# qq456cvb/CanonicalVoting

Hardware: AMD Instinct MI355X
Metric: scenes/sec (80k-pt synthetic scans) (higher is better)
Workload: dtype f32

## Files before the change

canonicalvoting_amd/_lib.py:

```python
import ctypes
import os
import threading

_HERE = os.path.dirname(os.path.abspath(__file__))
LIB_PATH = os.path.join(_HERE, "_C", "libcvhip.so")

c_float_p = ctypes.POINTER(ctypes.c_float)
c_int_p = ctypes.POINTER(ctypes.c_int)
c_i32_p = ctypes.POINTER(ctypes.c_int32)
c_i64_p = ctypes.POINTER(ctypes.c_int64)
vp = ctypes.c_void_p
ABI_VERSION = 6


class CvError(RuntimeError):
    pass


class DecodeParams(ctypes.Structure):
    _fields_ = [("thresh_high", ctypes.c_float), ("thresh_low", ctypes.c_float),
                ("valid_ratio", ctypes.c_float), ("elimination", ctypes.c_int),
                ("prob_thresh", ctypes.c_float), ("elim_hi_plus1", ctypes.c_int),
                ("max_iters", ctypes.c_int), ("err_thresh", ctypes.c_double)]


class ConvDesc(ctypes.Structure):
    _fields_ = [("in_", vp), ("n_in", ctypes.c_longlong), ("in_ld", ctypes.c_int), ("cin", ctypes.c_int),
                ("weight", vp), ("K", ctypes.c_int), ("cout", ctypes.c_int), ("nbr", vp),
                ("n_out", ctypes.c_longlong), ("scale", vp), ("shift", vp), ("residual", vp),
                ("res_ld", ctypes.c_int), ("relu", ctypes.c_int), ("out", vp), ("out_ld", ctypes.c_int),
                ("flavour", ctypes.c_int), ("ws", vp), ("ws_bytes", ctypes.c_size_t), ("row_perm", vp),
                ("j_begin", ctypes.c_int), ("j_end", ctypes.c_int), ("acc_in", vp), ("acc_ld", ctypes.c_int),
                ("perm_groups", ctypes.c_int), ("plan_ent", vp), ("plan_cnt", vp),
                ("weight_packed", vp), ("weight_x6", vp), ("in2", vp), ("in2_ld", ctypes.c_int), ("cin2", ctypes.c_int),
                ("weight2_x6", vp), ("perm_has_map", ctypes.c_int), ("weight_pieces", ctypes.c_int),
                ("acc_scale", ctypes.c_float), ("range_flag", vp), ("in_hl", ctypes.c_int), ("out_hl", ctypes.c_int),
                ("res_hl", ctypes.c_int), ("split_tickets", vp), ("acc_scale_dev", vp), ("valid_words", vp)]


class SceneMaps(ctypes.Structure):
    _fields_ = [("stem", ctypes.c_longlong), ("out", ctypes.c_longlong), ("down", ctypes.c_longlong * 4),
                ("k3", ctypes.c_longlong * 5), ("up", ctypes.c_longlong * 4), ("mask_perm", ctypes.c_longlong * 5),
                ("up_perm", ctypes.c_longlong * 4), ("scratch", ctypes.c_longlong), ("bitmap", ctypes.c_longlong)]


class ScenePlanLayout(ctypes.Structure):
    _fields_ = [("cap", ctypes.c_longlong), ("perm", ctypes.c_longlong), ("inv", ctypes.c_longlong),
                ("coords", ctypes.c_longlong * 5), ("vals", ctypes.c_longlong * 5), ("counts", ctypes.c_longlong),
                ("arena", ctypes.c_longlong), ("int_words", ctypes.c_longlong), ("key_words", ctypes.c_longlong),
                ("sort_ws_bytes", ctypes.c_size_t), ("levels_ws_bytes", ctypes.c_size_t)]


NET_MAP_SLOTS, NET_PERM_SLOTS = 15, 9


class NetBuf(ctypes.Structure):
    _fields_ = [("level", ctypes.c_int), ("channels", ctypes.c_int), ("rows_level", ctypes.c_int), ("hl", ctypes.c_int)]


class NetOp(ctypes.Structure):
    _fields_ = [("in_buf", ctypes.c_int), ("in_col", ctypes.c_int), ("cin", ctypes.c_int),
                ("out_buf", ctypes.c_int), ("out_col", ctypes.c_int), ("cout", ctypes.c_int),
                ("res_buf", ctypes.c_int), ("res_col", ctypes.c_int), ("map", ctypes.c_int), ("K", ctypes.c_int),
                ("perm", ctypes.c_int), ("perm_groups", ctypes.c_int), ("relu", ctypes.c_int),
                ("weight", vp), ("scale", vp), ("shift", vp), ("weight_x6", vp), ("in2_buf", ctypes.c_int),
                ("in2_col", ctypes.c_int), ("cin2", ctypes.c_int), ("weight2_x6", vp), ("weight_pieces", ctypes.c_int), ("acc_scale", ctypes.c_float)]


class NetModelParams(ctypes.Structure):
    _fields_ = [("weight_x6", vp), ("weight2_x6", vp), ("scale", vp), ("shift", vp), ("acc_scale", ctypes.c_float),
                ("reserved", ctypes.c_int * 3)]


class SceneDesc(ctypes.Structure):
    _fields_ = [("d_coords4", vp), ("n", ctypes.c_longlong), ("d_feats", vp), ("feats_ld", ctypes.c_int), ("d_points", vp),
                ("res", ctypes.c_float), ("num_rots", ctypes.c_int), ("ops", vp), ("n_ops", ctypes.c_int), ("bufs", vp),
                ("n_bufs", ctypes.c_int), ("stem_k", ctypes.c_int), ("mask_groups", ctypes.c_int),
                ("masked_min_rows", ctypes.c_longlong), ("max_channels", ctypes.c_int),
                ("use_range_flag", ctypes.c_int),
                ("d_out_feats", vp), ("out_ld", ctypes.c_int), ("out_channels", ctypes.c_int), ("nclasses", ctypes.c_int),
                ("log_scale", ctypes.c_int), ("d_xyz_in", vp), ("d_scale_in", vp), ("d_prob_in", vp), ("d_class_in", vp),
                ("vote_algo", ctypes.c_int), ("decode", DecodeParams), ("max_candidates", ctypes.c_int),
                ("nms_threshold", ctypes.c_double), ("d_ws", vp), ("ws_bytes", ctypes.c_size_t), ("d_grids", vp),
                ("grid_capacity_floats", ctypes.c_size_t), ("h_pinned", vp), ("pinned_bytes", ctypes.c_size_t),
                ("h_cand_idx", vp), ("h_verdict", vp), ("h_boxes", vp), ("h_scores", vp), ("h_classes", vp), ("h_pick", vp),
                ("adaptive_split", ctypes.c_int), ("events", vp * 5),
                ("conv_split_target", ctypes.c_int), ("vote_part_records", ctypes.c_int), ("peak_quotients", ctypes.c_int)]


MAX_CATEGORIES = 16


class SceneSeparateDesc(ctypes.Structure):
    _fields_ = [("d_coords4", vp), ("n", ctypes.c_longlong), ("d_feats", vp), ("feats_ld", ctypes.c_int), ("d_points", vp),
                ("res", ctypes.c_float), ("num_rots", ctypes.c_int), ("num_models", ctypes.c_int),
                ("ops", vp), ("n_ops", vp), ("bufs", vp), ("n_bufs", vp),
                ("stem_k", ctypes.c_int), ("mask_groups", ctypes.c_int), ("masked_min_rows", ctypes.c_longlong),
                ("max_channels", ctypes.c_int), ("use_range_flag", ctypes.c_int),
                ("d_out_feats", vp), ("out_ld", ctypes.c_int), ("out_channels", ctypes.c_int), ("log_scale", ctypes.c_int),
                ("d_xyz_in", vp), ("d_scale_in", vp), ("d_prob_in", vp), ("vote_algo", ctypes.c_int), ("decode", DecodeParams),
                ("max_candidates", ctypes.c_int), ("nms_threshold", ctypes.c_double), ("d_ws", vp), ("ws_bytes", ctypes.c_size_t),
                ("h_pinned", vp), ("pinned_bytes", ctypes.c_size_t), ("h_cand_idx", vp), ("h_verdict", vp), ("h_boxes", vp),
                ("h_scores", vp), ("h_det_cat", vp), ("h_det_box", vp), ("events", vp * 5),
                ("conv_split_target", ctypes.c_int), ("vote_part_records", ctypes.c_int),
                ("models_per_pass", ctypes.c_int), ("d_model_params", vp)]


class SceneSeparateResult(ctypes.Structure):
    _fields_ = [("n_cand", ctypes.c_int * MAX_CATEGORIES), ("n_boxes", ctypes.c_int * MAX_CATEGORIES),
                ("truncated", ctypes.c_int * MAX_CATEGORIES), ("n_det", ctypes.c_int), ("range_flag", ctypes.c_int),
                ("duplicates", ctypes.c_int), ("out_of_window", ctypes.c_int), ("dims", ctypes.c_int * 3),
                ("corner", ctypes.c_float * 3), ("level_rows", ctypes.c_longlong * 5), ("needed_ws_bytes", ctypes.c_size_t),
                ("d_grid_obj", vp), ("d_grid_rot", vp), ("d_grid_scale", vp), ("d_xyz", vp), ("d_scale", vp), ("d_prob", vp),
                ("host_us", ctypes.c_float * 4)]


class PackJob(ctypes.Structure):
    _fields_ = [("w", vp), ("wp", vp), ("K", ctypes.c_int), ("cin", ctypes.c_int), ("cout", ctypes.c_int), ("trans", ctypes.c_int),
                ("scale_log2", ctypes.c_int), ("reserved", ctypes.c_int)]


class SceneResult(ctypes.Structure):
    _fields_ = [("n_cand", ctypes.c_int), ("n_boxes", ctypes.c_int), ("n_det", ctypes.c_int), ("truncated", ctypes.c_int),
                ("range_flag", ctypes.c_int), ("duplicates", ctypes.c_int), ("out_of_window", ctypes.c_int),
                ("scenes_in_flight", ctypes.c_int), ("dims", ctypes.c_int * 3), ("corner", ctypes.c_float * 3), ("level_rows", ctypes.c_longlong * 5),
                ("needed_ws_bytes", ctypes.c_size_t), ("needed_grid_floats", ctypes.c_size_t),
                ("d_grid_obj", vp), ("d_grid_rot", vp), ("d_grid_scale", vp), ("d_xyz", vp), ("d_scale", vp),
                ("d_prob", vp), ("d_class", vp), ("host_us", ctypes.c_float * 4)]


MAX_SCENES = 16


class DecodeSceneJob(ctypes.Structure):
    _fields_ = [("d_grid_obj", vp), ("d_grid_rot", vp), ("d_grid_scale", vp), ("dims", ctypes.c_int * 3),
                ("corner", ctypes.c_float * 3), ("row0", ctypes.c_int64), ("n", ctypes.c_int64)]


class ScenesDesc(ctypes.Structure):
    _fields_ = [("scene", SceneDesc), ("num_scenes", ctypes.c_int)]


class ScenesResult(ctypes.Structure):
    _fields_ = [("n_cand", ctypes.c_int * MAX_SCENES), ("n_boxes", ctypes.c_int * MAX_SCENES), ("n_det", ctypes.c_int * MAX_SCENES),
                ("truncated", ctypes.c_int * MAX_SCENES), ("dims", ctypes.c_int * 3 * MAX_SCENES),
                ("corner", ctypes.c_float * 3 * MAX_SCENES), ("row0", ctypes.c_longlong * MAX_SCENES),
                ("rows", ctypes.c_longlong * MAX_SCENES), ("d_grid_obj", vp * MAX_SCENES), ("d_grid_rot", vp * MAX_SCENES),
                ("d_grid_scale", vp * MAX_SCENES), ("range_flag", ctypes.c_int), ("duplicates", ctypes.c_int),
                ("out_of_window", ctypes.c_int), ("scenes_in_flight", ctypes.c_int), ("level_rows", ctypes.c_longlong * 5),
                ("needed_ws_bytes", ctypes.c_size_t), ("needed_grid_floats", ctypes.c_size_t),
                ("d_xyz", vp), ("d_scale", vp), ("d_prob", vp), ("d_class", vp), ("host_us", ctypes.c_float * 4)]


GATHER_MAX_JOBS = 8


class GatherJob(ctypes.Structure):
    _fields_ = [("d_src", vp), ("src_ld", ctypes.c_longlong), ("d_dst", vp), ("dst_ld", ctypes.c_longlong),
                ("width", ctypes.c_int), ("recentre_from", ctypes.c_int)]


class ScanRowsDesc(ctypes.Structure):
    _fields_ = [("d_coords4", vp), ("d_index", vp), ("n", ctypes.c_longlong), ("m_points", ctypes.c_longlong),
                ("d_points", vp), ("points_ld", ctypes.c_longlong), ("d_rgb", vp), ("d_owner", vp),
                ("d_minv", vp), ("d_model_scale", vp), ("d_model_cls", vp), ("n_models", ctypes.c_int),
                ("d_colour", vp), ("d_jitter", vp), ("n_clouds", ctypes.c_int),
                ("use_xyz", ctypes.c_int), ("recentre", ctypes.c_int),
                ("d_feats", vp), ("feats_ld", ctypes.c_longlong), ("d_xyz", vp), ("xyz_ld", ctypes.c_longlong),
                ("d_scale", vp), ("scale_ld", ctypes.c_longlong), ("d_cls", vp), ("cls_ld", ctypes.c_longlong)]


class SymLossDesc(ctypes.Structure):
    _fields_ = [("d_out", vp), ("n_rows", ctypes.c_longlong), ("ld", ctypes.c_longlong),
                ("d_rows", vp), ("d_pseg", vp), ("n_points", ctypes.c_longlong),
                ("d_seg_ptr", vp), ("d_pose_ptr", vp), ("d_tgt_ptr", vp), ("n_segments", ctypes.c_int), ("n_jobs", ctypes.c_int),
                ("d_targets", vp), ("n_targets", ctypes.c_longlong),
                ("d_urow", vp), ("d_uptr", vp), ("d_upoint", vp), ("n_urows", ctypes.c_int),
                ("w", ctypes.c_float * 3), ("xyz_factor", ctypes.c_float),
                ("d_loss", vp), ("d_pose_loss", vp), ("d_best", vp), ("d_seg_loss", vp),
                ("d_grad_loss", vp), ("d_grad", vp), ("grad_ld", ctypes.c_longlong),
                ("d_ws", vp), ("ws_bytes", ctypes.c_size_t)]


class RowLossDesc(ctypes.Structure):
    _fields_ = [("d_out", vp), ("n_rows", ctypes.c_longlong), ("ld", ctypes.c_longlong),
                ("d_labels", vp), ("d_xyz_labels", vp), ("d_scale_labels", vp),
                ("heads", ctypes.c_int), ("n_logits", ctypes.c_int), ("xyz_col", ctypes.c_int), ("scale_col", ctypes.c_int),
                ("logit_col", ctypes.c_int), ("obj_lo", ctypes.c_longlong), ("obj_hi", ctypes.c_longlong),
                ("with_xyz", ctypes.c_int), ("log_scale", ctypes.c_int), ("gather", ctypes.c_int), ("empty", ctypes.c_int),
                ("w", ctypes.c_float * 3), ("xyz_factor", ctypes.c_float), ("scale_factor", ctypes.c_float),
# ... 315 lines not shown
```

canonicalvoting_amd/csrc/conv_hd.hip:

```cpp
#include "cv_common.h"

#include <algorithm>

#include "sparse_conv_common.h"

using namespace cvsc;

namespace {

constexpr int hd_lds_bytes(int NB, int NW, int NSTG) {
    return NSTG * (NW * 4096 + 2 * NB * 32 * 64) + NW * 32 * 4 + (WP_NPRE + 1) * NW * 32 * 4 + NW * 4 + (HL_MAX_UNITS + 4) * 2;
}
constexpr int hd_blocks(int NB, int NW, int NSTG) {
    const int b = (160 * 1024) / hd_lds_bytes(NB, NW, NSTG);
    return b * NW > 32 ? 32 / NW : (b < 1 ? 1 : b);
}
template <int NB, int NW, int NSTG, class... MA>
__global__ __launch_bounds__(NW * 64, (hd_blocks(NB, NW, NSTG) * NW + 3) / 4) void conv_hd(ConvArgs a, MA... ma) {
    const unsigned by = model_enter(a, blockIdx.y, ma...);
    static_assert(NSTG == 2 || NSTG == 3, "two or three ring stages");
    constexpr int TMv = NW * 32, THv = NW * 64;
    constexpr int A_BYTES = NW * 4096, B_BYTES = 2 * NB * 32 * 64, STAGE = A_BYTES + B_BYTES;
    constexpr int B_INSTR = B_BYTES / 1024;
    constexpr int B_PER_WAVE = (B_INSTR + NW - 1) / NW;
    constexpr int EP_BYTES = NW * 32 * EP_LD * 4;
    static_assert(EP_BYTES <= NSTG * STAGE, "the epilogue tile aliases the ring");
    constexpr int OFF_ROWS = NSTG * STAGE, OFF_NBR = OFF_ROWS + TMv * 4, OFF_MASK = OFF_NBR + (WP_NPRE + 1) * TMv * 4,
                  OFF_UNITS = OFF_MASK + NW * 4,
                  LDS_TOTAL = OFF_UNITS + (HL_MAX_UNITS + 4) * 2;
    static_assert(LDS_TOTAL == hd_lds_bytes(NB, NW, NSTG) && LDS_TOTAL <= 160 * 1024, "LDS budget");
    __shared__ __attribute__((aligned(1024))) unsigned char lds[LDS_TOTAL];
    unsigned char* const sm = lds;
    int* const rows_s = reinterpret_cast<int*>(lds + OFF_ROWS);
    int (*const nbr_all)[TMv] = reinterpret_cast<int (*)[TMv]>(lds + OFF_NBR);
    unsigned* const wave_mask = reinterpret_cast<unsigned*>(lds + OFF_MASK);
    unsigned short* const units_s = reinterpret_cast<unsigned short*>(lds + OFF_UNITS);
    const int tid = threadIdx.x, lane = tid & 63, wave = tid >> 6;
    const int n0 = by * (NB * 32);
    const long long tile_id = tile_of(a);
    const int half = lane >> 5, l31 = lane & 31;
    const int nj = a.j_end - a.j_begin;
    const int nch = a.cin / KC;
    int u_lo, u_hi;
    if (a.perm_per_split) {
        u_lo = (int)((long long)nj * blockIdx.z / a.splits) * nch;
        u_hi = (int)((long long)nj * (blockIdx.z + 1) / a.splits) * nch;
    } else {
        u_lo = (int)((long long)nj * nch * blockIdx.z / a.splits);
        u_hi = (int)((long long)nj * nch * (blockIdx.z + 1) / a.splits);
    }
    const int j_first = a.j_begin + u_lo / nch, j_last = a.j_begin + (u_hi - 1) / nch;
    const int njl = u_hi > u_lo ? j_last - j_first + 1 : 0;
    const int nch2 = a.in2 ? a.cin2 / KC : 0;

    const int* perm = a.row_perm ? a.row_perm + (a.perm_per_split ? (long long)blockIdx.z * a.n_out : 0) : nullptr;
    if (tid < TMv) {
        const long long t = tile_id * TMv + tid;
        const int row = t < a.n_out ? (perm ? perm[t] : (int)t) : -1;
        rows_s[tid] = row;
        if (a.in2) nbr_all[njl][tid] = row;
    }
    {
        unsigned m = 0u;
        const int jg0 = a.j_begin + (int)((long long)nj * blockIdx.z / a.splits);
        for (int e = tid; e < njl * TMv; e += THv) {
            const int jj = e / TMv, t = e - jj * TMv;
            const long long pos = tile_id * TMv + t;
            int v = -1;
            if (pos < a.n_out) {
                if (a.nbr_perm) {
                    v = a.nbr_perm[((long long)blockIdx.z * a.n_out + pos) * a.nbr_perm_w + (j_first + jj - jg0)];
                } else {
                    const int row = perm ? perm[pos] : (int)pos;
                    v = a.nbr ? a.nbr[(long long)row * a.K + j_first + jj] : row;
                }
            }
            nbr_all[jj][t] = v;
            if (v >= 0) m |= 1u << jj;
        }
#pragma unroll
        for (int off = 32; off > 0; off >>= 1) m |= __shfl_xor(m, off);
        if (lane == 0) wave_mask[wave] = m;
    }
    __syncthreads();
    unsigned lm = 0u;
#pragma unroll
    for (int w = 0; w < NW; ++w) lm |= wave_mask[w];
    if (wave == 0) {
        const int n_first = u_hi - u_lo, n_second = nch2 > (int)blockIdx.z ? (nch2 - (int)blockIdx.z + a.splits - 1) / a.splits : 0;
        int cnt = 0;
        for (int base = 0; base < n_first + n_second; base += 64) {
            const int e = base + lane;
            int code = -1;
            if (e < n_first) {
                const int u = u_lo + e, q = u / nch;
                const int jj = a.j_begin + q - j_first;
                if ((lm >> jj) & 1u) code = (jj << 8) | (u - q * nch);
            } else if (e < n_first + n_second) {
                code = (njl << 8) | ((int)blockIdx.z + (e - n_first) * a.splits);
            }
            const unsigned long long bal = __ballot(code >= 0);
            if (code >= 0) units_s[cnt + __popcll(bal & ((1ull << lane) - 1ull))] = (unsigned short)code;
            cnt += __popcll(bal);
        }
        if (lane == 0) units_s[HL_MAX_UNITS] = (unsigned short)cnt;
    }
    __syncthreads();
    const int n_units = __builtin_amdgcn_readfirstlane((int)units_s[HL_MAX_UNITS]);
    if (n_units == 0 && a.gvalid) return;

    f32x16 acc[NB];
#pragma unroll
    for (int nb = 0; nb < NB; ++nb)
#pragma unroll
        for (int r = 0; r < 16; ++r) acc[nb][r] = 0.f;

    int b_src[B_PER_WAVE];
#pragma unroll
    for (int i = 0; i < B_PER_WAVE; ++i) {
        const int t = wave + i * NW;
        const int f = t * 64 + lane;
        const int pl = f / (NB * 32 * 4), rem = f - pl * (NB * 32 * 4);
        const int col = rem >> 2, slot = rem & 3;
        const int gc = min(n0 + col, a.cout - 1);
        b_src[i] = (pl * a.cout + gc) * 32 + ((slot ^ ((col >> 2) & 3)) << 3);
    }
    const unsigned slab_words = 2u * (unsigned)a.cout * 32u;
    const unsigned in_row_bytes = (unsigned)a.in_ld * 4u, in2_row_bytes = (unsigned)a.in2_ld * 4u;
    const unsigned char* const in_b = reinterpret_cast<const unsigned char*>(a.in);
    const unsigned char* const in2_b = reinterpret_cast<const unsigned char*>(a.in2);
    const int a_row = lane >> 3;
    unsigned a_piece[4];
#pragma unroll
    for (int q = 0; q < 4; ++q) a_piece[q] = (unsigned)(((lane & 7) ^ (((8 * q + a_row) >> 1) & 7)) << 4);

    bool live[NSTG];
#pragma unroll
    for (int q = 0; q < NSTG; ++q) live[q] = false;

    auto issue = [&](auto S, int k) -> int {
        constexpr int st = decltype(S)::value;
        const int code = __builtin_amdgcn_readfirstlane((int)units_s[k]);
        const int jj = code >> 8, c = code & 255;
        const bool second = jj == njl;
        int n_issued = 0;
        int src[4];
        bool any = false;
#pragma unroll
        for (int q = 0; q < 4; ++q) {
            src[q] = nbr_all[jj][wave * 32 + 8 * q + a_row];
            any |= src[q] >= 0;
        }
        const bool lv = __any(any);
        live[st] = lv;
        if (lv) {
            const unsigned rb_ = second ? in2_row_bytes : in_row_bytes;
            const unsigned char* const base = (second ? in2_b : in_b) + (unsigned)(c * 128);
#pragma unroll
            for (int q = 0; q < 4; ++q) {
                const unsigned char* g = src[q] >= 0 ? base + ((unsigned)src[q] * rb_ + a_piece[q]) : g_zero_chunk + a_piece[q];
                lds_dma16(g, sm + st * STAGE + wave * 4096 + q * 1024);
            }
            n_issued += 4;
        }
        const unsigned short* slab = second ? a.wp6_2 + (size_t)c * slab_words
                                            : a.wp6 + (size_t)((j_first + jj) * nch + c) * slab_words;
#pragma unroll
        for (int i = 0; i < B_PER_WAVE; ++i) {
            const int t = wave + i * NW;
            if (t < B_INSTR) {
                lds_dma16(slab + b_src[i], sm + st * STAGE + A_BYTES + t * 1024);
                ++n_issued;
            }
        }
        return n_issued;
    };
    const unsigned lds0 = (unsigned)(size_t)(lds_ptr_t)lds;
    const int bswz = (l31 >> 2) & 3, a_g = (l31 >> 1) & 7;
    unsigned a_off[4], b_off[2];
#pragma unroll
    for (int kk = 0; kk < 4; ++kk) a_off[kk] = lds0 + (unsigned)(wave * 4096 + l31 * 128 + (((2 * kk + half) ^ a_g) << 4));
#pragma unroll
    for (int ks = 0; ks < 2; ++ks) b_off[ks] = lds0 + (unsigned)(A_BYTES + l31 * 64 + (((2 * ks + half) ^ bswz) << 4));
    auto compute = [&](auto S) {
        constexpr int st = decltype(S)::value;
#pragma unroll
        for (int ks = 0; ks < 2; ++ks) {
            const unsigned aa0 = a_off[ks] + st * STAGE, aa1 = a_off[2 + ks] + st * STAGE, ab = b_off[ks] + st * STAGE;
            u32x4v A0, A1, B0[NB], B1[NB];
            hd_read_frags<NB>(aa0, aa1, ab, A0, A1, B0, B1);
            const f16x8 a0 = __builtin_bit_cast(f16x8, A0), a1 = __builtin_bit_cast(f16x8, A1);
#pragma unroll
            for (int nb = 0; nb < NB; ++nb) {
                const f16x8 b0 = __builtin_bit_cast(f16x8, B0[nb]), b1 = __builtin_bit_cast(f16x8, B1[nb]);
                acc[nb] = __builtin_amdgcn_mfma_f32_32x32x16_f16(a0, b1, acc[nb], 0, 0, 0);
                acc[nb] = __builtin_amdgcn_mfma_f32_32x32x16_f16(a1, b0, acc[nb], 0, 0, 0);
                acc[nb] = __builtin_amdgcn_mfma_f32_32x32x16_f16(a0, b0, acc[nb], 0, 0, 0);
            }
        }
    };
    typedef std::integral_constant<int, 0> S0;
    typedef std::integral_constant<int, 1> S1;
    typedef std::integral_constant<int, 2> S2;
    if constexpr (NSTG == 3) {
        int pend1 = 0;
        if (n_units > 0) issue(S0{}, 0);
        if (n_units > 1) pend1 = issue(S1{}, 1);
        auto step = [&](auto S, auto SP, int k) {
            constexpr int st = decltype(S)::value;
            wait_vmcnt_dyn(__builtin_amdgcn_readfirstlane(k + 1 < n_units ? pend1 : 0));
            __builtin_amdgcn_s_barrier();
            if (k + 2 < n_units) pend1 = issue(SP, k + 2);
            else pend1 = 0;
            if (live[st]) compute(S);
        };
#pragma unroll 1
        for (int k = 0; k < n_units; k += 3) {
            step(S0{}, S2{}, k);
            if (k + 1 >= n_units) break;
            step(S1{}, S0{}, k + 1);
            if (k + 2 >= n_units) break;
            step(S2{}, S1{}, k + 2);
        }
    } else {
        if (n_units > 0) issue(S0{}, 0);
        auto step = [&](auto S, auto SN, int k) {
            constexpr int st = decltype(S)::value;
            wait_vmcnt_le<0>();
            __builtin_amdgcn_s_barrier();
            if (k + 1 < n_units) issue(SN, k + 1);
            if (live[st]) compute(S);
        };
#pragma unroll 1
        for (int k = 0; k < n_units; k += 2) {
            step(S0{}, S1{}, k);
            if (k + 1 >= n_units) break;
            step(S1{}, S0{}, k + 1);
        }
    }
    wait_vmcnt_le<0>();
    __syncthreads();
    model_epilogue(a, blockIdx.y, ma...);
    {
        const float sc = a.acc_scale_dev ? a.acc_scale * *a.acc_scale_dev : a.acc_scale;
#pragma unroll
        for (int nb = 0; nb < NB; ++nb)
#pragma unroll
            for (int r = 0; r < 16; ++r) acc[nb][r] *= sc;
    }
    float (*ep)[EP_LD] = reinterpret_cast<float (*)[EP_LD]>(sm + wave * 32 * EP_LD * 4);
    ConvArgs ae = a;
    ae.tickets = nullptr;
#pragma unroll
    for (int nb = 0; nb < NB; ++nb) epilogue_store_wide(ae, acc[nb], rows_s + wave * 32, n0 + nb * 32, lane, ep);
}


}

void cvsc::launch_conv_hd(const ConvArgs& a, int nb, int hd_shape, const ModelArgs* ma, dim3 grid, hipStream_t st) {
    with_nb<3>(nb, [&](auto nbc) {
        constexpr int NB = decltype(nbc)::value;
        if (hd_shape == 1) with_models(ma, [&](auto... m) { conv_hd<NB, 4, 2, decltype(m)...><<<grid, 256, 0, st>>>(a, m...); });
        else if (hd_shape == 2) with_models(ma, [&](auto... m) { conv_hd<NB, 8, 2, decltype(m)...><<<grid, 512, 0, st>>>(a, m...); });
        else with_models(ma, [&](auto... m) { conv_hd<NB, 8, 3, decltype(m)...><<<grid, 512, 0, st>>>(a, m...); });
    });
}
```

canonicalvoting_amd/csrc/conv_hl.hip:

```cpp
#include "cv_common.h"

#include <algorithm>

#include "sparse_conv_common.h"

using namespace cvsc;

namespace {

constexpr int hl_blocks(int NB) { return NB <= 3 ? 4 : 2; }
template <int NB, class... MA>
__global__ __attribute__((amdgpu_waves_per_eu(hl_blocks(NB), 8)))
__launch_bounds__(THREADS, hl_blocks(NB)) void conv_hl(ConvArgs a, MA... ma) {
    const unsigned by = model_enter(a, blockIdx.y, ma...);
    constexpr int NS = 2, NW = THREADS / 64;
    constexpr int B_BYTES = 2 * NB * 32 * 64, EP_BYTES = NW * 32 * EP_LD * 4;
    constexpr int SM_BYTES = NS * B_BYTES > EP_BYTES ? NS * B_BYTES : EP_BYTES;
    __shared__ __attribute__((aligned(16))) unsigned char sm[SM_BYTES];
    __shared__ int rows_s[TM];
    __shared__ int nbr_all[WP_NPRE + 1][TM];
    __shared__ unsigned wave_mask[NW];
    __shared__ unsigned short units_s[HL_MAX_UNITS + 4];
    const int tid = threadIdx.x, lane = tid & 63, wave = tid >> 6;
    const int n0 = by * (NB * 32);
    const long long tile_id = tile_of(a);
    const int half = lane >> 5, l31 = lane & 31;
    const int nj = a.j_end - a.j_begin;
    const int nch = a.cin / KC;
    int u_lo, u_hi;
    if (a.perm_per_split) {
        u_lo = (int)((long long)nj * blockIdx.z / a.splits) * nch;
        u_hi = (int)((long long)nj * (blockIdx.z + 1) / a.splits) * nch;
    } else {
        u_lo = (int)((long long)nj * nch * blockIdx.z / a.splits);
        u_hi = (int)((long long)nj * nch * (blockIdx.z + 1) / a.splits);
    }
    const int j_first = a.j_begin + u_lo / nch, j_last = a.j_begin + (u_hi - 1) / nch;
    const int njl = u_hi > u_lo ? j_last - j_first + 1 : 0;
    const int nch2 = a.in2 ? a.cin2 / KC : 0;

    const int* perm = a.row_perm ? a.row_perm + (a.perm_per_split ? (long long)blockIdx.z * a.n_out : 0) : nullptr;
    if (tid < TM) {
        const long long t = tile_id * TM + tid;
        const int row = t < a.n_out ? (perm ? perm[t] : (int)t) : -1;
        rows_s[tid] = row;
        if (a.in2) nbr_all[njl][tid] = row;
    }
    {
        unsigned m = 0u;
        const int jg0 = a.j_begin + (int)((long long)nj * blockIdx.z / a.splits);
        for (int e = tid; e < njl * TM; e += THREADS) {
            const int jj = e / TM, t = e - jj * TM;
            const long long pos = tile_id * TM + t;
            int v = -1;
            if (pos < a.n_out) {
                if (a.nbr_perm) {
                    v = a.nbr_perm[((long long)blockIdx.z * a.n_out + pos) * a.nbr_perm_w + (j_first + jj - jg0)];
                } else {
                    const int row = perm ? perm[pos] : (int)pos;
                    v = a.nbr ? a.nbr[(long long)row * a.K + j_first + jj] : row;
                }
            }
            nbr_all[jj][t] = v;
            if (v >= 0) m |= 1u << jj;
        }
#pragma unroll
        for (int off = 32; off > 0; off >>= 1) m |= __shfl_xor(m, off);
        if (lane == 0) wave_mask[wave] = m;
    }
    __syncthreads();
    unsigned lm = 0u;
#pragma unroll
    for (int w = 0; w < NW; ++w) lm |= wave_mask[w];
    if (wave == 0) {
        const int n_first = u_hi - u_lo, n_second = nch2 > (int)blockIdx.z ? (nch2 - (int)blockIdx.z + a.splits - 1) / a.splits : 0;
        int cnt = 0;
        for (int base = 0; base < n_first + n_second; base += 64) {
            const int e = base + lane;
            int code = -1;
            if (e < n_first) {
                const int u = u_lo + e, q = u / nch;
                const int jj = a.j_begin + q - j_first;
                if ((lm >> jj) & 1u) code = (jj << 8) | (u - q * nch);
            } else if (e < n_first + n_second) {
                code = (njl << 8) | ((int)blockIdx.z + (e - n_first) * a.splits);
            }
            const unsigned long long bal = __ballot(code >= 0);
            if (code >= 0) units_s[cnt + __popcll(bal & ((1ull << lane) - 1ull))] = (unsigned short)code;
            cnt += __popcll(bal);
        }
        if (lane == 0) units_s[HL_MAX_UNITS] = (unsigned short)cnt;
    }
    __syncthreads();
    const int n_units = __builtin_amdgcn_readfirstlane((int)units_s[HL_MAX_UNITS]);
    if (n_units == 0 && a.gvalid) return;

    f32x16 acc[NB];
#pragma unroll
    for (int nb = 0; nb < NB; ++nb)
#pragma unroll
        for (int r = 0; r < 16; ++r) acc[nb][r] = 0.f;

    constexpr int B_U4 = 2 * NB * 32 * 4;
    constexpr int B_PER = (B_U4 + THREADS - 1) / THREADS;
    int b_src[B_PER], b_dst[B_PER];
#pragma unroll
    for (int i = 0; i < B_PER; ++i) {
        const int f = tid + i * THREADS;
        const int p = f / (NB * 32 * 4), rem = f - p * (NB * 32 * 4);
        const int col = rem >> 2, ch = rem & 3;
        b_src[i] = (f < B_U4 && n0 + col < a.cout) ? (p * a.cout + n0 + col) * 32 + ch * 8 : -1;
        b_dst[i] = f < B_U4 ? (p * NB * 32 + col) * 64 + ((ch ^ ((col >> 2) & 3)) << 4) : -1;
    }
    const unsigned slab_words = 2u * (unsigned)a.cout * 32u;
    const int my_row = wave * 32 + l31;
    const unsigned in_row_bytes = (unsigned)a.in_ld * 4u, in2_row_bytes = (unsigned)a.in2_ld * 4u;
    const unsigned char* const in_b = reinterpret_cast<const unsigned char*>(a.in);
    const unsigned char* const in2_b = reinterpret_cast<const unsigned char*>(a.in2);

    uint4 ra[NS][4], rb[NS][B_PER];
    bool live[NS];
#pragma unroll
    for (int q = 0; q < NS; ++q) live[q] = false;
    auto load = [&](auto S, int k) {
        constexpr int sl = decltype(S)::value;
        const int code = __builtin_amdgcn_readfirstlane((int)units_s[k]);
        const int jj = code >> 8, c = code & 255;
        const bool second = jj == njl;
        const int src = nbr_all[jj][my_row];
        live[sl] = __any(src >= 0);
        if (src >= 0) {
            const unsigned off = (unsigned)src * (second ? in2_row_bytes : in_row_bytes) + (unsigned)(c * 128 + half * 16);
            const unsigned char* p = (second ? in2_b : in_b) + off;
            ra[sl][0] = *reinterpret_cast<const uint4*>(p);
            ra[sl][1] = *reinterpret_cast<const uint4*>(p + 32);
            ra[sl][2] = *reinterpret_cast<const uint4*>(p + 64);
            ra[sl][3] = *reinterpret_cast<const uint4*>(p + 96);
        } else {
#pragma unroll
            for (int q = 0; q < 4; ++q) ra[sl][q] = make_uint4(0u, 0u, 0u, 0u);
        }
        const unsigned short* slab = second ? a.wp6_2 + (size_t)c * slab_words
                                            : a.wp6 + (size_t)((j_first + jj) * nch + c) * slab_words;
#pragma unroll
        for (int i = 0; i < B_PER; ++i)
            rb[sl][i] = b_src[i] >= 0 ? *reinterpret_cast<const uint4*>(slab + b_src[i]) : make_uint4(0u, 0u, 0u, 0u);
    };
    auto stage_b = [&](auto S, int toff) {
        constexpr int sl = decltype(S)::value;
#pragma unroll
        for (int i = 0; i < B_PER; ++i)
            if (b_dst[i] >= 0) *reinterpret_cast<uint4*>(sm + toff + b_dst[i]) = rb[sl][i];
    };
    const int b_rd = l31 * 64;
    const int bswz = (l31 >> 2) & 3;
    auto compute = [&](auto S, int toff) {
        constexpr int sl = decltype(S)::value;
        const unsigned char* Bb = sm + toff + b_rd;
        uint4 (&fa)[4] = ra[sl];
#pragma unroll
        for (int ks = 0; ks < 2; ++ks) {
            const int piece = ((2 * ks + half) ^ bswz) << 4;
            const f16x8 a0 = __builtin_bit_cast(f16x8, fa[ks]), a1 = __builtin_bit_cast(f16x8, fa[2 + ks]);
#pragma unroll
            for (int nb = 0; nb < NB; ++nb) {
                const f16x8 b0 = *reinterpret_cast<const f16x8*>(Bb + nb * 32 * 64 + piece);
                const f16x8 b1 = *reinterpret_cast<const f16x8*>(Bb + (NB * 32 + nb * 32) * 64 + piece);
                acc[nb] = __builtin_amdgcn_mfma_f32_32x32x16_f16(a0, b1, acc[nb], 0, 0, 0);
                acc[nb] = __builtin_amdgcn_mfma_f32_32x32x16_f16(a1, b0, acc[nb], 0, 0, 0);
                acc[nb] = __builtin_amdgcn_mfma_f32_32x32x16_f16(a0, b0, acc[nb], 0, 0, 0);
                if constexpr (NB >= 3) asm volatile("" ::: "memory");
            }
        }
    };
    typedef std::integral_constant<int, 0> S0;
    typedef std::integral_constant<int, 1> S1;
    if (n_units > 0) load(S0{}, 0);
    if (n_units > 1) load(S1{}, 1);
    if (n_units > 0) stage_b(S0{}, 0);
    auto step = [&](auto S, auto SN, int k) {
        constexpr int sl = decltype(S)::value;
        __syncthreads();
        if (k + 1 < n_units) stage_b(SN, decltype(SN)::value * B_BYTES);
        if (live[sl]) compute(S, sl * B_BYTES);
        if (k + 2 < n_units) load(S, k + 2);
    };
#pragma unroll 1
    for (int k = 0; k < n_units; k += 2) {
        step(S0{}, S1{}, k);
        if (k + 1 >= n_units) break;
        step(S1{}, S0{}, k + 1);
    }
    __syncthreads();
    model_epilogue(a, blockIdx.y, ma...);
    {
        const float sc = a.acc_scale_dev ? a.acc_scale * *a.acc_scale_dev : a.acc_scale;
#pragma unroll
        for (int nb = 0; nb < NB; ++nb)
#pragma unroll
            for (int r = 0; r < 16; ++r) acc[nb][r] *= sc;
    }
    float (*ep)[EP_LD] = reinterpret_cast<float (*)[EP_LD]>(sm + wave * 32 * EP_LD * 4);
#pragma unroll
    for (int nb = 0; nb < NB; ++nb) epilogue_store_wide(a, acc[nb], rows_s + wave * 32, n0 + nb * 32, lane, ep);
    if (a.splits > 1 && a.tickets) {
        __shared__ int last_flag;
        asm volatile("s_waitcnt vmcnt(0)" ::: "memory");
        __syncthreads();
        int* ticket = a.tickets + tile_id * gridDim.y + by;
        if (tid == 0) {
            const int old = __hip_atomic_fetch_add(ticket, 1, __ATOMIC_RELAXED, __HIP_MEMORY_SCOPE_AGENT);
            last_flag = old == a.splits - 1;
            if (last_flag) __builtin_amdgcn_fence(__ATOMIC_ACQUIRE, "agent");
        }
        __syncthreads();
        if (!last_flag) return;
        if (tid == 0) *ticket = 0;
        const long long plane = a.n_out * (long long)a.cout;
#pragma unroll
        for (int nb = 0; nb < NB; ++nb) {
            const int col = n0 + nb * 32 + (lane & 7) * 4;
            if (col >= a.cout) continue;
#pragma unroll
            for (int it = 0; it < 4; ++it) {
                const int row = rows_s[wave * 32 + (lane >> 3) + 8 * it];
                if (row < 0) continue;
                const float* p = a.partial + (long long)row * a.cout + col;
                float4 sq[4];
#pragma unroll
                for (int q = 0; q < 4; ++q) sq[q] = make_float4(0.f, 0.f, 0.f, 0.f);
                for (int k0 = 0; k0 < a.splits; k0 += 4) {
#pragma unroll
                    for (int q = 0; q < 4; ++q)
                        if (k0 + q < a.splits) {
                            const float4 v = *reinterpret_cast<const float4*>(p + (long long)(k0 + q) * plane);
                            sq[q].x += v.x; sq[q].y += v.y; sq[q].z += v.z; sq[q].w += v.w;
                        }
                }
                const float4 x = make_float4(sq[0].x + sq[1].x + sq[2].x + sq[3].x, sq[0].y + sq[1].y + sq[2].y + sq[3].y,
                                             sq[0].z + sq[1].z + sq[2].z + sq[3].z, sq[0].w + sq[1].w + sq[2].w + sq[3].w);
                epilogue_apply4(a, row, col, x);
            }
        }
    }
}

}

void cvsc::launch_conv_hl(const ConvArgs& a, int nb, const ModelArgs* ma, dim3 grid, hipStream_t st) {
    with_nb<4>(nb, [&](auto nbc) {
        constexpr int NB = decltype(nbc)::value;
        with_models(ma, [&](auto... m) { conv_hl<NB, decltype(m)...><<<grid, THREADS, 0, st>>>(a, m...); });
    });
}
```

canonicalvoting_amd/csrc/conv_rows.hip:

```cpp
#include "cv_common.h"

#include <algorithm>

#include "sparse_conv_common.h"

using namespace cvsc;

namespace {

template <int NB, bool VEC>
__global__ __launch_bounds__(THREADS) void conv_rows(ConvArgs a) {
    __shared__ float A_s[KC][A_LD];
    __shared__ float B_s[KC][NB * 32];
    __shared__ int nbr_s[TM];
    __shared__ int rows_s[TM];
    __shared__ __attribute__((aligned(16))) float ep_s[4][32][EP_LD];
    const int tid = threadIdx.x, lane = tid & 63, wave = tid >> 6;
    const int n0 = blockIdx.y * (NB * 32);

    if (tid < TM) {
        const long long t = tile_of(a) * TM + tid;
        const int* perm = a.row_perm ? a.row_perm + (a.perm_per_split ? (long long)blockIdx.z * a.n_out : 0) : nullptr;
        rows_s[tid] = t < a.n_out ? (perm ? perm[t] : (int)t) : -1;
    }
    __syncthreads();

    f32x16 acc[NB];
#pragma unroll
    for (int nb = 0; nb < NB; ++nb)
#pragma unroll
        for (int r = 0; r < 16; ++r) acc[nb][r] = 0.f;

    auto compute = [&]() {
#pragma unroll
        for (int kk = 0; kk < KC; kk += 2) {
            const float av = A_s[kk + (lane >> 5)][wave * 32 + (lane & 31)];
#pragma unroll
            for (int nb = 0; nb < NB; ++nb) {
                const float bv = B_s[kk + (lane >> 5)][nb * 32 + (lane & 31)];
                acc[nb] = __builtin_amdgcn_mfma_f32_32x32x2f32(av, bv, acc[nb], 0, 0, 0);
            }
        }
    };

    const int nj = a.j_end - a.j_begin;
    if (VEC) {
        const int a_col = (tid & 7) * 4;
        const int a_row = tid >> 3;
        constexpr int B_F4 = KC * NB * 32 / 4;
        constexpr int B_PER = (B_F4 + THREADS - 1) / THREADS;
        const int nch = a.cin / KC;
        int u_lo, u_hi;
        if (a.perm_per_split) {
            u_lo = (int)((long long)nj * blockIdx.z / a.splits) * nch;
            u_hi = (int)((long long)nj * (blockIdx.z + 1) / a.splits) * nch;
        } else {
            u_lo = (int)((long long)nj * nch * blockIdx.z / a.splits);
            u_hi = (int)((long long)nj * nch * (blockIdx.z + 1) / a.splits);
        }
        const int j_first = a.j_begin + u_lo / nch, j_last = a.j_begin + (u_hi - 1) / nch;
        for (int j = j_first; j <= j_last && u_hi > u_lo; ++j) {
            const int kc_begin = (j == j_first ? u_lo % nch : 0) * KC;
            const int kc_end = (j == j_last ? (u_hi - 1) % nch + 1 : nch) * KC;
            int my = -1;
            if (tid < TM) {
                const int row = rows_s[tid];
                if (row >= 0) {
                    if (a.nbr_perm) {
                        const long long tile_id = (long long)gridDim.x - 1 - blockIdx.x;
                        my = a.nbr_perm[((long long)blockIdx.z * a.n_out + tile_id * TM + tid) * a.nbr_perm_w +
                                        (j - (a.j_begin + (int)((long long)nj * blockIdx.z / a.splits)))];
                    } else
                        my = a.nbr ? a.nbr[(long long)row * a.K + j] : row;
                }
                nbr_s[tid] = my;
            }
            if (!__syncthreads_or(my >= 0)) continue;
            const bool wave_live = __any(nbr_s[wave * 32 + (lane & 31)] >= 0);
            float4 ra[4], rb[B_PER];
            auto load = [&](int kc) {
#pragma unroll
                for (int i = 0; i < 4; ++i) {
                    const int src = nbr_s[a_row + 32 * i];
                    ra[i] = src >= 0 ? *reinterpret_cast<const float4*>(a.in + (long long)src * a.in_ld + kc + a_col)
                                     : make_float4(0.f, 0.f, 0.f, 0.f);
                }
#pragma unroll
                for (int i = 0; i < B_PER; ++i) {
                    const int f = tid + i * THREADS;
                    if (f < B_F4) {
                        const int kr = f / (NB * 8), c4 = (f % (NB * 8)) * 4;
                        const int col = n0 + c4;
                        const float* wp = a.w + ((long long)j * a.cin + kc + kr) * a.cout + col;
                        if (col + 3 < a.cout) rb[i] = *reinterpret_cast<const float4*>(wp);
                        else {
                            rb[i].x = col < a.cout ? wp[0] : 0.f;
                            rb[i].y = col + 1 < a.cout ? wp[1] : 0.f;
                            rb[i].z = col + 2 < a.cout ? wp[2] : 0.f;
                            rb[i].w = 0.f;
                        }
                    }
                }
            };
            auto stage = [&]() {
#pragma unroll
                for (int i = 0; i < 4; ++i) {
                    const int r = a_row + 32 * i;
                    A_s[a_col + 0][r] = ra[i].x; A_s[a_col + 1][r] = ra[i].y;
                    A_s[a_col + 2][r] = ra[i].z; A_s[a_col + 3][r] = ra[i].w;
                }
#pragma unroll
                for (int i = 0; i < B_PER; ++i) {
                    const int f = tid + i * THREADS;
                    if (f < B_F4) {
                        const int kr = f / (NB * 8), c4 = (f % (NB * 8)) * 4;
                        *reinterpret_cast<float4*>(&B_s[kr][c4]) = rb[i];
                    }
                }
            };
            load(kc_begin);
            for (int kc = kc_begin; kc < kc_end; kc += KC) {
                __syncthreads();
                stage();
                __syncthreads();
                if (kc + KC < kc_end) load(kc + KC);
                if (wave_live) compute();
            }
            __syncthreads();
        }
    } else {
        const int k0 = a.j_begin * a.cin, ktot = a.j_end * a.cin;
        const int nchunks = (ktot - k0 + KC - 1) / KC;
        const int c_lo = (int)((long long)nchunks * blockIdx.z / a.splits);
        const int c_hi = (int)((long long)nchunks * (blockIdx.z + 1) / a.splits);
        for (int kc = k0 + c_lo * KC; kc < k0 + c_hi * KC; kc += KC) {
            __syncthreads();
            for (int e = tid; e < KC * TM; e += THREADS) {
                const int kk = e / TM, r = e % TM;
                const int kf = kc + kk;
                float v = 0.f;
                const int row = rows_s[r];
                if (kf < ktot && row >= 0) {
                    const int j = kf / a.cin, c = kf - j * a.cin;
                    const int src = a.nbr ? a.nbr[(long long)row * a.K + j] : row;
                    if (src >= 0) v = a.in[(long long)src * a.in_ld + c];
                }
                A_s[kk][r] = v;
            }
            for (int e = tid; e < KC * NB * 32; e += THREADS) {
                const int kr = e / (NB * 32), c = e % (NB * 32);
                const int kf = kc + kr, col = n0 + c;
                B_s[kr][c] = (kf < ktot && col < a.cout) ? a.w[(long long)kf * a.cout + col] : 0.f;
            }
            __syncthreads();
            compute();
        }
    }
    if (a.wide) {
#pragma unroll
        for (int nb = 0; nb < NB; ++nb)
            epilogue_store_wide(a, acc[nb], rows_s + wave * 32, n0 + nb * 32, lane, ep_s[wave]);
    } else {
#pragma unroll
        for (int nb = 0; nb < NB; ++nb)
            epilogue_store(a, acc[nb], rows_s + wave * 32, n0 + nb * 32 + (lane & 31), lane);
    }
}

}

void cvsc::launch_conv_rows(const ConvArgs& a, int nb, bool vec, dim3 grid, hipStream_t st) {
    with_nb<4>(nb, [&](auto nbc) {
        constexpr int NB = decltype(nbc)::value;
        if (vec) conv_rows<NB, true><<<grid, THREADS, 0, st>>>(a);
        else conv_rows<NB, false><<<grid, THREADS, 0, st>>>(a);
    });
}
```

canonicalvoting_amd/csrc/conv_rows_wp.hip:

```cpp
#include "cv_common.h"

#include <algorithm>

#include "sparse_conv_common.h"

using namespace cvsc;

namespace {


template <int NB, int P, int NPRE = WP_NPRE>
__global__ __launch_bounds__(THREADS, (NB >= 3 ? 3 : NB == 2 ? 4 : 5)) void conv_rows_wp(ConvArgs a) {
    constexpr int A_BYTES = P * TM * 64, B_BYTES = P * NB * 32 * 64, EP_BYTES = 4 * 32 * EP_LD * 4;
    constexpr int SM_BYTES = A_BYTES + 2 * B_BYTES > EP_BYTES ? A_BYTES + 2 * B_BYTES : EP_BYTES;
    __shared__ __attribute__((aligned(16))) unsigned char sm[SM_BYTES];
    __shared__ int rows_s[TM];
    __shared__ int nbr_all[NPRE + 1][TM];
    __shared__ unsigned live_mask;
    unsigned char* const A_h = sm;
    unsigned char* const B_h = sm + A_BYTES;
    const int tid = threadIdx.x, lane = tid & 63, wave = tid >> 6;
    const int n0 = blockIdx.y * (NB * 32);

    const long long tile_id = tile_of(a);
// ... 43 lines not shown
                    acc[nb] = __builtin_amdgcn_mfma_f32_32x32x16_f16(a0, b1, acc[nb], 0, 0, 0);
                    acc[nb] = __builtin_amdgcn_mfma_f32_32x32x16_f16(a1, b0, acc[nb], 0, 0, 0);
                    acc[nb] = __builtin_amdgcn_mfma_f32_32x32x16_f16(a0, b0, acc[nb], 0, 0, 0);
                }
            }
        }
    };

    const int nj = a.j_end - a.j_begin;
    const int a_col = (lane & 7) * 4;
    const int a_row = wave * 32 + (lane >> 3);
    constexpr int B_U4 = P * NB * 32 * 4;
    constexpr int B_PER = (B_U4 + THREADS - 1) / THREADS;
    const int nch = a.cin / KC;
    int u_lo, u_hi;
    if (a.perm_per_split) {
        u_lo = (int)((long long)nj * blockIdx.z / a.splits) * nch;
        u_hi = (int)((long long)nj * (blockIdx.z + 1) / a.splits) * nch;
    } else {
        u_lo = (int)((long long)nj * nch * blockIdx.z / a.splits);
        u_hi = (int)((long long)nj * nch * (blockIdx.z + 1) / a.splits);
    }
    const int j_first = a.j_begin + u_lo / nch, j_last = a.j_begin + (u_hi - 1) / nch;
    const int njl = u_hi > u_lo ? j_last - j_first + 1 : 0;
    auto map_entry = [&](int t, int j) {
        const int row = rows_s[t];
        if (row < 0) return -1;
        if (a.nbr_perm) {
            return a.nbr_perm[((long long)blockIdx.z * a.n_out + tile_id * TM + t) * a.nbr_perm_w +
                              (j - (a.j_begin + (int)((long long)nj * blockIdx.z / a.splits)))];
        }
        return a.nbr ? a.nbr[(long long)row * a.K + j] : row;
    };
    {
        unsigned m = 0u;
        for (int e = tid; e < njl * TM; e += THREADS) {
            const int jj = e / TM, t = e - jj * TM;
            const int v = map_entry(t, j_first + jj);
            nbr_all[jj][t] = v;
            if (v >= 0) m |= 1u << jj;
        }
#pragma unroll
        for (int off = 32; off > 0; off >>= 1) m |= __shfl_xor(m, off);
        if (lane == 0 && m) atomicOr(&live_mask, m);
        if (a.in2 && tid < TM) nbr_all[njl][tid] = rows_s[tid];
    }
    __syncthreads();
    const unsigned lm = live_mask;

    float4 ra[4];
    uint4 rb[B_PER];
    float in_max = 0.f;
    const int c_first = u_lo - (u_lo / nch) * nch, c_last = u_hi > u_lo ? (u_hi - 1) - ((u_hi - 1) / nch) * nch + 1 : 0;
    auto skip_dead = [&](int& j, int& c) {
#pragma unroll 1
        while (j <= j_last && !((lm >> (j - j_first)) & 1u)) { ++j; c = 0; }
    };
    const int nch2 = a.in2 ? a.cin2 / KC : 0;
    const int j_second = j_last + 1, j_done = j_last + 2;
    auto advance = [&](int& j, int& c) {
        if (j <= j_last) {
            if (++c >= (j == j_last ? c_last : nch)) { ++j; c = 0; skip_dead(j, c); }
            if (j > j_last) { j = j_second; c = blockIdx.z; }
        } else {
            c += a.splits;
        }
        if (j == j_second && c >= nch2) j = j_done;
    };
    auto load = [&](int j, int c) {
        const bool second = j == j_second;
        const int kc = c * KC;
        const int* nb_j = nbr_all[j - j_first];
        const float* src_base = second ? a.in2 : a.in;
        const int src_ld = second ? a.in2_ld : a.in_ld;
#pragma unroll
        for (int i = 0; i < 4; ++i) {
            const int src = nb_j[a_row + 8 * i];
            ra[i] = src >= 0 ? *reinterpret_cast<const float4*>(src_base + (long long)src * src_ld + kc + a_col)
                             : make_float4(0.f, 0.f, 0.f, 0.f);
        }
        const unsigned short* slab = second ? a.wp6_2 + (long long)c * P * a.cout * 32
                                            : a.wp6 + (long long)(j * nch + c) * P * a.cout * 32;
#pragma unroll
        for (int i = 0; i < B_PER; ++i) {
            const int f = tid + i * THREADS;
            if (f < B_U4) {
                const int p = f / (NB * 32 * 4), rem = f - p * (NB * 32 * 4);
                const int col = rem >> 2, ch = rem & 3;
                rb[i] = (n0 + col < a.cout)
                            ? *reinterpret_cast<const uint4*>(slab + ((long long)p * a.cout + n0 + col) * 32 + ch * 8)
                            : make_uint4(0u, 0u, 0u, 0u);
            }
        }
    };
    auto stage = [&](unsigned char* Bb) {
#pragma unroll
        for (int i = 0; i < 4; ++i) {
            const int r = a_row + 8 * i;
            unsigned h0 = 0, m0 = 0, l0 = 0, h1 = 0, m1 = 0, l1 = 0;
            unsigned char* dst = A_h + r * 64 + ((((a_col >> 3) ^ ((r >> 2) & 3))) << 4) + ((a_col & 7) << 1);
            if constexpr (P == 1) {
                *reinterpret_cast<uint2*>(dst) = make_uint2(cvt_pk_bf16(ra[i].x, ra[i].y), cvt_pk_bf16(ra[i].z, ra[i].w));
            } else if constexpr (P == 3) {
                split3(ra[i].x, ra[i].y, h0, m0, l0);
                split3(ra[i].z, ra[i].w, h1, m1, l1);
                *reinterpret_cast<uint2*>(dst) = make_uint2(h0, h1);
                *reinterpret_cast<uint2*>(dst + TM * 64) = make_uint2(m0, m1);
                *reinterpret_cast<uint2*>(dst + 2 * TM * 64) = make_uint2(l0, l1);
            } else {
                in_max = fmaxf(fmaxf(in_max, fmaxf(fabsf(ra[i].x), fabsf(ra[i].y))), fmaxf(fabsf(ra[i].z), fabsf(ra[i].w)));
                split2h(ra[i].x, ra[i].y, h0, l0);
                split2h(ra[i].z, ra[i].w, h1, l1);
                *reinterpret_cast<uint2*>(dst) = make_uint2(h0, h1);
                *reinterpret_cast<uint2*>(dst + TM * 64) = make_uint2(l0, l1);
            }
        }
#pragma unroll
        for (int i = 0; i < B_PER; ++i) {
            const int f = tid + i * THREADS;
            if (f < B_U4) {
                const int p = f / (NB * 32 * 4), rem = f - p * (NB * 32 * 4);
                const int col = rem >> 2, ch = rem & 3;
                *reinterpret_cast<uint4*>(Bb + (p * NB * 32 + col) * 64 + ((ch ^ ((col >> 2) & 3)) << 4)) = rb[i];
            }
        }
    };
    int j = j_first, c = c_first, buf = 0;
    if (njl > 0) skip_dead(j, c); else j = j_last + 1;
    if (j > j_last) { j = j_second; c = blockIdx.z; if (c >= nch2) j = j_done; }
    if (j < j_done) load(j, c);
#pragma unroll 1
    while (j < j_done) {
        unsigned char* Bb = B_h + buf * B_BYTES;
        stage(Bb);
        __syncthreads();
        const bool wave_live = __any(nbr_all[j - j_first][wave * 32 + l31] >= 0);
        advance(j, c);
        if (j < j_done) load(j, c);
        if (wave_live) compute(Bb);
        buf ^= 1;
    }
    __syncthreads();
    if constexpr (P == 2) {
        if (in_max > 65000.f && a.range_flag) *a.range_flag = 1;
        const float k = a.acc_scale;
#pragma unroll
        for (int nb = 0; nb < NB; ++nb)
#pragma unroll
            for (int r = 0; r < 16; ++r) acc[nb][r] *= k;
    }
    float (*ep)[EP_LD] = reinterpret_cast<float (*)[EP_LD]>(sm + wave * 32 * EP_LD * 4);
    if (a.wide) {
#pragma unroll
        for (int nb = 0; nb < NB; ++nb) epilogue_store_wide(a, acc[nb], rows_s + wave * 32, n0 + nb * 32, lane, ep);
    } else {
#pragma unroll
        for (int nb = 0; nb < NB; ++nb)
            epilogue_store(a, acc[nb], rows_s + wave * 32, n0 + nb * 32 + (lane & 31), lane);
    }
}

}

void cvsc::launch_conv_rows_wp(const ConvArgs& a, int nb, int pieces, bool npre_big, dim3 grid, hipStream_t st) {
    with_nb<4>(nb, [&](auto nbc) {
        constexpr int NB = decltype(nbc)::value;
        if (npre_big) {
            if (pieces == 2) conv_rows_wp<NB, 2, WP_NPRE_BIG><<<grid, THREADS, 0, st>>>(a);
            else if (pieces == 1) conv_rows_wp<NB, 1, WP_NPRE_BIG><<<grid, THREADS, 0, st>>>(a);
            else conv_rows_wp<NB, 3, WP_NPRE_BIG><<<grid, THREADS, 0, st>>>(a);
        } else {
            if (pieces == 2) conv_rows_wp<NB, 2><<<grid, THREADS, 0, st>>>(a);
            else if (pieces == 1) conv_rows_wp<NB, 1><<<grid, THREADS, 0, st>>>(a);
            else conv_rows_wp<NB, 3><<<grid, THREADS, 0, st>>>(a);
        }
    });
}
```

canonicalvoting_amd/csrc/net_exec.cpp:

```cpp
#include <algorithm>
#include <mutex>
#include <unordered_map>
#include <vector>

#include "cv_common.h"

namespace {

struct Slot { char* ptr; int ld; long long rows; int ext; };

struct NetModels {
    int K;
    const void* const* const* ext_ptr;
    size_t arena_stride, ws_stride;
    const cv_net_model_params* d_params;
    int params_ld;
};

int net_run(const cv_net_op* ops, int n_ops, const cv_net_buf* bufs, int n_bufs, const long long* level_rows, int n_levels,
            void* d_arena, size_t arena_bytes, const void* const* ext_ptr, const int* ext_ld, const int32_t* const* maps,
            int n_maps, const int32_t* const* perms, int n_perms, void* d_ws, size_t ws_bytes, int32_t* range_flag,
            const NetModels* nm, bool plan_maps, void* stream);

}
// ... 288 lines not shown
    cv_net_model_params* t = static_cast<cv_net_model_params*>(h_params);
    for (int k = 0; k < n_ops; ++k)
        for (int m = 0; m < K; ++m) {
            const cv_net_op& o = ops[m][k];
            t[(size_t)k * K + m] = {o.weight_x6, o.weight2_x6, o.scale, o.shift, o.acc_scale != 0.f ? o.acc_scale : 1.f, {0, 0, 0}};
        }
    return CV_OK;
}

size_t cv_net_models_arena_bytes(const cv_net_buf* bufs, int n_bufs, const long long* level_rows, int n_levels, int K) {
    if (K < 1 || K > CV_MAX_CATEGORIES) return 0;
    return (size_t)K * cv_net_arena_bytes(bufs, n_bufs, level_rows, n_levels);
}

size_t cv_net_models_workspace_bytes(size_t one_model_bytes, int K) {
    if (K < 1 || K > CV_MAX_CATEGORIES) return 0;
    return (size_t)(K - 1) * cv_align_up(one_model_bytes, 256) + one_model_bytes;
}

int cv_net_run_models_f32(const cv_net_op* const* ops, const cv_net_buf* const* bufs, int n_ops, int n_bufs, int K,
                          const long long* level_rows, int n_levels, void* d_arena, size_t arena_bytes,
                          const void* const* const* ext_ptr, const int* ext_ld, const int32_t* const* maps, int n_maps,
                          const int32_t* const* perms, int n_perms, void* d_ws, size_t ws_bytes, int32_t* range_flag,
                          const void* d_params, int params_ld, void* stream) {
    return cv_net_run_models_ex(ops, bufs, n_ops, n_bufs, K, level_rows, n_levels, d_arena, arena_bytes, ext_ptr, ext_ld, maps, n_maps,
                                perms, n_perms, d_ws, ws_bytes, range_flag, d_params, params_ld,  false, stream);
}

}

int cv_net_run_models_ex(const cv_net_op* const* ops, const cv_net_buf* const* bufs, int n_ops, int n_bufs, int K,
                         const long long* level_rows, int n_levels, void* d_arena, size_t arena_bytes,
                         const void* const* const* ext_ptr, const int* ext_ld, const int32_t* const* maps, int n_maps,
                         const int32_t* const* perms, int n_perms, void* d_ws, size_t ws_bytes, int32_t* range_flag,
                         const void* d_params, int params_ld, bool plan_maps, void* stream) {
    CV_REQUIRE(K >= 1 && K <= CV_MAX_CATEGORIES, CV_EINVAL, "number of models out of range (%d, 1..%d)", K, CV_MAX_CATEGORIES);
    CV_REQUIRE(ops && bufs && level_rows && d_arena && ext_ptr && n_ops > 0 && n_bufs > 0 && n_levels > 0, CV_EINVAL,
               "bad network program arguments");
    CV_REQUIRE(d_params, CV_EINVAL, "null model parameter table (cv_net_models_params_fill)");
    CV_REQUIRE(params_ld >= K, CV_EINVAL, "params_ld (%d) is smaller than the number of models (%d)", params_ld, K);
    for (int m = 0; m < K; ++m)
        CV_REQUIRE(ops[m] && bufs[m] && ext_ptr[m], CV_EINVAL, "model %d: null program, buffer list or pointer table", m);
    for (int m = 1; m < K; ++m) {
        for (int i = 0; i < n_bufs; ++i) {
            const cv_net_buf &x = bufs[0][i], &y = bufs[m][i];
            CV_REQUIRE(x.level == y.level && x.channels == y.channels && x.rows_level == y.rows_level && x.hl == y.hl, CV_EINVAL,
                       "buffer %d of model %d differs from model 0's: the programs are not structurally identical", i, m);
        }
        for (int k = 0; k < n_ops; ++k) {
            const cv_net_op &x = ops[0][k], &y = ops[m][k];
            const bool same = x.in_buf == y.in_buf && x.in_col == y.in_col && x.cin == y.cin && x.out_buf == y.out_buf &&
                              x.out_col == y.out_col && x.cout == y.cout && x.res_buf == y.res_buf && x.res_col == y.res_col &&
                              x.map == y.map && x.K == y.K && x.perm == y.perm && x.perm_groups == y.perm_groups &&
                              x.relu == y.relu && x.in2_buf == y.in2_buf && x.in2_col == y.in2_col && x.cin2 == y.cin2 &&
                              x.weight_pieces == y.weight_pieces && !x.weight == !y.weight && !x.scale == !y.scale &&
                              !x.shift == !y.shift && !x.weight_x6 == !y.weight_x6 && !x.weight2_x6 == !y.weight2_x6;
            CV_REQUIRE(same, CV_EINVAL, "op %d of model %d differs from model 0's: the programs are not structurally identical", k, m);
        }
    }
    for (int k = 0; k < n_ops; ++k)
        for (int m = 0; m < K; ++m) {
            const cv_net_op& o = ops[m][k];
            CV_REQUIRE(o.weight_pieces == 2, CV_EINVAL, "op %d: the model axis runs fp16-pair programs only (weight_pieces == 2)", k);
            CV_REQUIRE(((reinterpret_cast<uintptr_t>(o.scale) | reinterpret_cast<uintptr_t>(o.shift) |
                         reinterpret_cast<uintptr_t>(o.weight_x6) | reinterpret_cast<uintptr_t>(o.weight2_x6)) & 15) == 0, CV_EINVAL,
                       "op %d of model %d: scale, shift and packed weights must be 16-byte aligned", k, m);
        }
    const size_t arena_one = cv_net_arena_bytes(bufs[0], n_bufs, level_rows, n_levels);
    CV_REQUIRE(arena_bytes >= (size_t)K * arena_one, CV_ENOMEM, "arena too small (cv_net_models_arena_bytes)");
    const size_t ws_stride = K > 1 ? (ws_bytes / (size_t)K) & ~(size_t)255 : 0;
    const size_t ws_one = K > 1 ? ws_stride : ws_bytes;
    NetModels nm = {K, ext_ptr, arena_one, ws_stride, static_cast<const cv_net_model_params*>(d_params), params_ld};
    return net_run(ops[0], n_ops, bufs[0], n_bufs, level_rows, n_levels, d_arena, arena_one, ext_ptr[0], ext_ld, maps, n_maps,
                   perms, n_perms, d_ws, ws_one, range_flag, &nm, plan_maps, stream);
}

namespace {

int net_run(const cv_net_op* ops, int n_ops, const cv_net_buf* bufs, int n_bufs, const long long* level_rows, int n_levels,
            void* d_arena, size_t arena_bytes, const void* const* ext_ptr, const int* ext_ld, const int32_t* const* maps,
            int n_maps, const int32_t* const* perms, int n_perms, void* d_ws, size_t ws_bytes, int32_t* range_flag,
            const NetModels* nm, bool plan_maps, void* stream) {
    CV_REQUIRE(ops && bufs && level_rows && d_arena && n_ops > 0 && n_bufs > 0 && n_levels > 0, CV_EINVAL,
               "bad network program arguments");
    CV_REQUIRE(arena_bytes >= cv_net_arena_bytes(bufs, n_bufs, level_rows, n_levels), CV_ENOMEM, "arena too small");
    std::vector<Slot> slot((size_t)n_bufs);
    {
        CvCarver cv(d_arena);
        int ext = 0;
        for (int i = 0; i < n_bufs; ++i) {
            const int lv = bufs[i].level;
            if (lv < 0 || lv >= n_levels) {
                CV_REQUIRE(ext_ptr && ext_ld && ext_ptr[ext], CV_EINVAL, "external buffer %d has no pointer", ext);
                slot[i] = {static_cast<char*>(const_cast<void*>(ext_ptr[ext])), ext_ld[ext], bufs[i].rows_level >= 0 &&
                           bufs[i].rows_level < n_levels ? level_rows[bufs[i].rows_level] : 0, ext};
                if (nm)
                    for (int m = 1; m < nm->K; ++m)
                        CV_REQUIRE(nm->ext_ptr[m][ext], CV_EINVAL, "external buffer %d of model %d has no pointer", ext, m);
                ++ext;
            } else {
                slot[i] = {reinterpret_cast<char*>(cv.take<float>((size_t)level_rows[lv] * bufs[i].channels)),
                           bufs[i].channels, level_rows[lv], -1};
            }
        }
    }
    for (int k = 0; k < n_ops; ++k) {
        const cv_net_op& o = ops[k];
        CV_REQUIRE(o.in_buf >= 0 && o.in_buf < n_bufs && o.out_buf >= 0 && o.out_buf < n_bufs &&
                       o.res_buf < n_bufs && o.map < n_maps && o.perm < n_perms, CV_EINVAL, "op %d: bad slot", k);
        const Slot& in = slot[o.in_buf];
        const Slot& out = slot[o.out_buf];
        cv_conv_desc d = {};
        d.in_hl = bufs[o.in_buf].hl;
        d.out_hl = bufs[o.out_buf].hl;
        d.res_hl = o.res_buf >= 0 ? bufs[o.res_buf].hl : 0;
        CV_REQUIRE(o.in2_buf < 0 || bufs[o.in2_buf].hl == d.in_hl, CV_EINVAL, "op %d: both sources must share a format", k);
        d.in = reinterpret_cast<const float*>(in.ptr) + o.in_col;
        d.n_in = in.rows;
        d.in_ld = in.ld;
        d.cin = o.cin;
        d.weight = o.weight;
        d.weight_x6 = o.weight_x6;
        d.weight_pieces = o.weight_pieces;
        d.acc_scale = o.acc_scale;
        d.range_flag = (o.weight_pieces == 2 || d.out_hl) ? range_flag : nullptr;
        if (o.in2_buf >= 0) {
            CV_REQUIRE(o.in2_buf < n_bufs, CV_EINVAL, "op %d: bad second-source slot", k);
            d.in2 = reinterpret_cast<const float*>(slot[o.in2_buf].ptr) + o.in2_col;
            d.in2_ld = slot[o.in2_buf].ld;
            d.cin2 = o.cin2;
            d.weight2_x6 = o.weight2_x6;
        }
        d.K = o.K;
        d.cout = o.cout;
        d.nbr = o.map >= 0 ? maps[o.map] : nullptr;
        d.n_out = out.rows;
        d.scale = o.scale;
        d.shift = o.shift;
        if (o.res_buf >= 0) {
            d.residual = reinterpret_cast<const float*>(slot[o.res_buf].ptr) + o.res_col;
            d.res_ld = slot[o.res_buf].ld;
        }
        d.relu = o.relu;
        d.out = reinterpret_cast<float*>(out.ptr) + o.out_col;
        d.out_ld = out.ld;
        d.ws = d_ws;
        d.ws_bytes = ws_bytes;
        const int32_t* perm = o.perm >= 0 ? perms[o.perm] : nullptr;
        if (perm) {
            d.row_perm = perm;
            d.perm_groups = o.perm_groups;
            d.perm_has_map = o.perm_groups > 1;
            if (plan_maps && d.perm_has_map && o.K == 27 && d.nbr) d.valid_words = d.nbr + out.rows * 27;
        }
        int rc;
        if (nm) {
            CvConvModels cm = {};
            cm.models = nm->K;
            cm.d_params = nm->d_params + (size_t)k * nm->params_ld;
            cm.ws_stride = (long long)nm->ws_stride;
            auto stride_of = [&](int buf, long long* stride) -> int {
                const int e = slot[buf].ext;
                if (e < 0) { *stride = (long long)nm->arena_stride; return CV_OK; }
                for (int m = 1; m < nm->K; ++m)
                    CV_REQUIRE(nm->ext_ptr[m][e] == nm->ext_ptr[0][e], CV_EINVAL,
                               "op %d: the external buffer it reads must be the same tensor for every model (model %d differs)", k, m);
                *stride = 0;
                return CV_OK;
            };
            if ((rc = stride_of(o.in_buf, &cm.in_stride)) != CV_OK) return rc;
            if (o.in2_buf >= 0 && (rc = stride_of(o.in2_buf, &cm.in2_stride)) != CV_OK) return rc;
            if (o.res_buf >= 0 && (rc = stride_of(o.res_buf, &cm.res_stride)) != CV_OK) return rc;
            if (out.ext >= 0) {
                cm.out_ext = 1;
                for (int m = 0; m < nm->K; ++m) {
                    float* p = reinterpret_cast<float*>(const_cast<void*>(nm->ext_ptr[m][out.ext])) + o.out_col;
                    CV_REQUIRE((reinterpret_cast<uintptr_t>(p) & 15) == 0, CV_EINVAL, "op %d: output of model %d is not 16-byte aligned", k, m);
                    cm.ext_out[m] = p;
                }
            } else {
                cm.out_stride = (long long)nm->arena_stride;
            }
            rc = cv_sp_conv_models_f32(&d, &cm, stream);
        } else {
            rc = cv_sp_conv_f32(&d, stream);
        }
        if (rc != CV_OK) return rc;
    }
    return CV_OK;
}

}
```

canonicalvoting_amd/csrc/sparse_conv.hip:

```cpp
#include "cv_common.h"

#include <atomic>
#include <cstring>
#include <type_traits>
#include <utility>

#include "sparse_conv_common.h"

using namespace cvsc;

namespace {

template <int CIN, class... MA>
__global__ __launch_bounds__(THREADS, (CIN <= 3 ? 3 : 1)) void conv_stem_mfma(ConvArgs a, MA... ma) {
    model_enter_y(a, ma...);
    constexpr int G = 8;
    constexpr int W_BYTES = G * CIN * 2 * 1024;
    constexpr int EP_BYTES = 4 * 32 * EP_LD * 4;
    constexpr int SM_BYTES = W_BYTES > EP_BYTES ? W_BYTES : EP_BYTES;
    __shared__ __attribute__((aligned(16))) unsigned char w_s[SM_BYTES];
    __shared__ int rows_s[TM];
    const int tid = threadIdx.x, lane = tid & 63, wave = tid >> 6;
    const int half = lane >> 5, l31 = lane & 31;
    const long long r0 = (long long)blockIdx.x * TM;
    for (int f = tid; f < W_BYTES / 16; f += THREADS)
        reinterpret_cast<uint4*>(w_s)[f] = reinterpret_cast<const uint4*>(a.wp6)[f];
    if (tid < TM) rows_s[tid] = r0 + tid < a.n_out ? (int)(r0 + tid) : -1;
    const long long row = r0 + wave * 32 + l31;
    const bool have = row < a.n_out;
    const int K = a.K;
    const int* __restrict__ mrow = a.nbr + (have ? row : 0) * (long long)K;
    f32x16 acc;
#pragma unroll
    for (int r = 0; r < 16; ++r) acc[r] = 0.f;
    float in_max = 0.f;
    int m[G][8];
#pragma unroll
    for (int g = 0; g < G; ++g)
#pragma unroll
        for (int i = 0; i < 8; ++i) {
            const int j = g * 16 + half * 8 + i;
            m[g][i] = (have && j < K) ? mrow[j] : -1;
        }
    float x0[8][CIN], x1[8][CIN];
    auto gather = [&](const int* mg, float (*x)[CIN]) {
#pragma unroll
        for (int i = 0; i < 8; ++i) {
            if (mg[i] >= 0) {
                const float* p = a.in + (long long)mg[i] * a.in_ld;
#pragma unroll
                for (int ci = 0; ci < CIN; ++ci) x[i][ci] = p[ci];
            } else {
#pragma unroll
                for (int ci = 0; ci < CIN; ++ci) x[i][ci] = 0.f;
            }
        }
    };
    gather(m[0], x1);
    __syncthreads();
#pragma unroll
    for (int g = 0; g < G; ++g) {
        bool any = false;
#pragma unroll
        for (int i = 0; i < 8; ++i) {
#pragma unroll
            for (int ci = 0; ci < CIN; ++ci) x0[i][ci] = x1[i][ci];
            any |= m[g][i] >= 0;
        }
        if (g + 1 < G) gather(m[g + 1], x1);
        if (__any(any)) {
#pragma unroll
            for (int ci = 0; ci < CIN; ++ci) {
                unsigned h[4], l[4];
#pragma unroll
                for (int q = 0; q < 4; ++q) {
                    in_max = fmaxf(in_max, fmaxf(fabsf(x0[2 * q][ci]), fabsf(x0[2 * q + 1][ci])));
                    split2h(x0[2 * q][ci], x0[2 * q + 1][ci], h[q], l[q]);
                }
                const f16x8 a0 = __builtin_bit_cast(f16x8, make_uint4(h[0], h[1], h[2], h[3]));
                const f16x8 a1 = __builtin_bit_cast(f16x8, make_uint4(l[0], l[1], l[2], l[3]));
                const unsigned char* wb = w_s + ((g * CIN + ci) * 2) * 1024 + (l31 * 2 + half) * 16;
                const f16x8 b0 = *reinterpret_cast<const f16x8*>(wb);
                const f16x8 b1 = *reinterpret_cast<const f16x8*>(wb + 1024);
                acc = __builtin_amdgcn_mfma_f32_32x32x16_f16(a0, b1, acc, 0, 0, 0);
                acc = __builtin_amdgcn_mfma_f32_32x32x16_f16(a1, b0, acc, 0, 0, 0);
                acc = __builtin_amdgcn_mfma_f32_32x32x16_f16(a0, b0, acc, 0, 0, 0);
            }
        }
    }
    if (in_max > 65000.f && a.range_flag) *a.range_flag = 1;
    {
        const float sc = a.acc_scale_dev ? a.acc_scale * *a.acc_scale_dev : a.acc_scale;
#pragma unroll
        for (int r = 0; r < 16; ++r) acc[r] *= sc;
    }
    __syncthreads();
    float (*ep)[EP_LD] = reinterpret_cast<float (*)[EP_LD]>(w_s + wave * 32 * EP_LD * 4);
    epilogue_store_wide(a, acc, rows_s + wave * 32, 0, lane, ep);
}

template <class... MA>
__global__ __launch_bounds__(256) void conv_finish(ConvArgs a, MA... ma) {
    model_enter_y(a, ma...);
    __shared__ float4 red[4][64];
    const int q = threadIdx.x >> 6, l = threadIdx.x & 63;
    const long long total4 = a.n_out * (long long)a.cout / 4;
    const long long total = a.n_out * (long long)a.cout;
    for (long long base = blockIdx.x * 64ll; base < total4; base += (long long)gridDim.x * 64) {
        const long long e4 = base + l;
        float4 s = make_float4(0.f, 0.f, 0.f, 0.f);
        if (e4 < total4) {
            const float4* p = reinterpret_cast<const float4*>(a.partial) + e4;
#pragma unroll 4
            for (int k = q; k < a.splits; k += 4) {
                const float4 v = partial_load4(p + (long long)k * (total / 4));
                s.x += v.x; s.y += v.y; s.z += v.z; s.w += v.w;
            }
        }
        red[q][l] = s;
        __syncthreads();
        if (q == 0 && e4 < total4) {
            float v[4] = {red[0][l].x + red[1][l].x + red[2][l].x + red[3][l].x,
                          red[0][l].y + red[1][l].y + red[2][l].y + red[3][l].y,
                          red[0][l].z + red[1][l].z + red[2][l].z + red[3][l].z,
                          red[0][l].w + red[1][l].w + red[2][l].w + red[3][l].w};
            const long long e = e4 * 4;
            const long long row = e / a.cout;
            const int col = (int)(e - row * a.cout);
            if (a.wide) {
                epilogue_apply4(a, row, col, make_float4(v[0], v[1], v[2], v[3]));
            } else {
#pragma unroll
                for (int i = 0; i < 4; ++i) epilogue_apply1(a, row, col + i, v[i]);
            }
        }
        __syncthreads();
    }
}

constexpr int FINISH_SMALL_MAX = 16;
template <int SMAX> struct FinishMasks { unsigned m[SMAX]; };

template <int SMAX, class IDX, class... MA>
__global__ __launch_bounds__(256) void conv_finish_small(ConvArgs a, FinishMasks<SMAX> gm, MA... ma) {
    model_enter_y(a, ma...);
    const IDX cq = (IDX)(a.cout >> 2);
    const IDX total4 = (IDX)a.n_out * cq;
    const IDX e4 = (IDX)blockIdx.x * (IDX)256 + (IDX)threadIdx.x;
    if (e4 >= total4) return;
    const IDX row = e4 / cq;
    const int col = (int)(e4 - row * cq) * 4;
    const unsigned w = a.gvalid ? (unsigned)a.gvalid[row] : ~0u;
    const float4* p = reinterpret_cast<const float4*>(a.partial) + e4;
    float4 pv[SMAX];
#pragma unroll
    for (int k = 0; k < SMAX; ++k)
        pv[k] = (w & gm.m[k]) ? partial_load4(p + (long long)k * (long long)total4) : make_float4(0.f, 0.f, 0.f, 0.f);
    float4 sq[4];
#pragma unroll
    for (int q = 0; q < 4; ++q) sq[q] = make_float4(0.f, 0.f, 0.f, 0.f);
#pragma unroll
    for (int k = 0; k < SMAX; ++k)
        if (k < a.splits) { sq[k & 3].x += pv[k].x; sq[k & 3].y += pv[k].y; sq[k & 3].z += pv[k].z; sq[k & 3].w += pv[k].w; }
    const float4 x = make_float4(sq[0].x + sq[1].x + sq[2].x + sq[3].x, sq[0].y + sq[1].y + sq[2].y + sq[3].y,
                                 sq[0].z + sq[1].z + sq[2].z + sq[3].z, sq[0].w + sq[1].w + sq[2].w + sq[3].w);
    epilogue_apply4(a, (long long)row, col, x);
}

template <class... MA>
__global__ __launch_bounds__(256) void conv_finish_scalar(ConvArgs a, MA... ma) {
    model_enter_y(a, ma...);
    const long long total = a.n_out * (long long)a.cout;
    for (long long t = blockIdx.x * 256ll + threadIdx.x; t < total; t += (long long)gridDim.x * 256) {
        const long long row = t / a.cout;
        const int col = (int)(t - row * a.cout);
        float v = 0.f;
        for (int sidx = 0; sidx < a.splits; ++sidx) v += a.partial[sidx * total + t];
        epilogue_apply1(a, row, col, v);
    }
}

template <int SMAX, class IDX>
void launch_finish_small(const ConvArgs& a, hipStream_t st, const ModelArgs* ma, int models) {
    FinishMasks<SMAX> gm;
    for (int k = 0; k < SMAX; ++k) {
        gm.m[k] = k < a.splits ? ~0u : 0u;
        if (a.gvalid && k < a.splits) {
            const int jb = a.K * k / a.splits, je = a.K * (k + 1) / a.splits;
            gm.m[k] = (unsigned)(((1ull << je) - 1) & ~((1ull << jb) - 1));
        }
    }
    const long long items = a.n_out * (long long)a.cout / 4;
    const dim3 grid((unsigned)((items + 255) / 256), (unsigned)models);
    with_models(ma, [&](auto... m) { conv_finish_small<SMAX, IDX, decltype(m)...><<<grid, 256, 0, st>>>(a, gm, m...); });
}

std::atomic<int> g_ablation{0};
int launch_finish(const ConvArgs& a, hipStream_t st, const ModelArgs* ma, int models) {
    if (g_ablation.load(std::memory_order_relaxed) & 1) return CV_OK;
    const long long total = a.n_out * (long long)a.cout;
    const auto grid = [&](long long items, int per_block, long long cap) {
        return dim3((unsigned)std::min<long long>((items + per_block - 1) / per_block, cap), (unsigned)models);
    };
    if (a.wide && a.splits <= FINISH_SMALL_MAX) {
        const auto with_idx = [&](auto smax) {
            if (total < (1ll << 31)) launch_finish_small<smax.value, unsigned>(a, st, ma, models);
            else launch_finish_small<smax.value, long long>(a, st, ma, models);
        };
        if (a.splits <= 4) with_idx(std::integral_constant<int, 4>{});
        else if (a.splits <= 8) with_idx(std::integral_constant<int, 8>{});
        else with_idx(std::integral_constant<int, FINISH_SMALL_MAX>{});
    } else if (a.cout % 4 == 0)
        with_models(ma, [&](auto... m) { conv_finish<decltype(m)...><<<grid(total / 4, 64, 8192), 256, 0, st>>>(a, m...); });
    else
        with_models(ma, [&](auto... m) { conv_finish_scalar<decltype(m)...><<<grid(total, 256, 4096), 256, 0, st>>>(a, m...); });
    CV_LAUNCH_CHECK();
    return CV_OK;
}

std::atomic<long long> g_opt_zskip{getenv("CV_ZSKIP") ? atoll(getenv("CV_ZSKIP")) : 1};
std::atomic<long long> g_zskip_launches{0};
std::atomic<long long> g_opt_hd_mask{getenv("CV_HD") ? atoll(getenv("CV_HD")) : 4};
std::atomic<long long> g_opt_hd_min_rows{getenv("CV_HD_MIN_ROWS") ? atoll(getenv("CV_HD_MIN_ROWS")) : 16384};
std::atomic<long long> g_opt_hd_shape{getenv("CV_HD_SHAPE") ? atoll(getenv("CV_HD_SHAPE")) : 2};

int launch_rows(ConvArgs a, const int NB, bool vec, hipStream_t st, ModelArgs* ma, int models) {
    dim3 grid((unsigned)((a.n_out + TM - 1) / TM), (unsigned)((a.cout + NB * 32 - 1) / (NB * 32)),
              (unsigned)a.splits);
    int per_wg = 0;
    if (vec) {
        const int nj_wp = a.j_end - a.j_begin, nch_wp = a.cin / KC;
        for (int z = 0; z < a.splits; ++z) {
            long long lo, hi;
            if (a.perm_per_split) {
                lo = (long long)nj_wp * z / a.splits * nch_wp;
                hi = (long long)nj_wp * (z + 1) / a.splits * nch_wp;
            } else {
                lo = (long long)nj_wp * nch_wp * z / a.splits;
                hi = (long long)nj_wp * nch_wp * (z + 1) / a.splits;
            }
            if (hi > lo) per_wg = std::max(per_wg, (int)((hi - 1) / nch_wp - lo / nch_wp + 1));
        }
    }
    if (ma) {
        CV_REQUIRE(a.in_hl && !a.tickets, CV_EINVAL,
                   "the model axis runs fp16-pair programs on hl buffers only (no fp32 / bf16 convolution, no split_tickets)");
        ma->ncb = (int)grid.y;
        grid.y *= (unsigned)models;
    }
    if (a.in_hl) {
        CV_REQUIRE(per_wg * (a.cin / KC) + (a.in2 ? a.cin2 / KC : 0) <= HL_MAX_UNITS, CV_EINVAL,
                   "hl-format convolution: more than %d units per workgroup (Cin too wide)", HL_MAX_UNITS);
        CV_REQUIRE(vec && a.wp6 && a.pieces == 2 && a.wide && per_wg <= WP_NPRE && NB <= 4, CV_EINVAL,
                   "hl-format input needs the fp16-pair weights, Cin %% 32 == 0, 16-byte aligned operands and at most %d "
                   "kernel offsets per workgroup", WP_NPRE);
        const int hd_mask = (int)g_opt_hd_mask.load(std::memory_order_relaxed);
        const long long hd_min_rows = g_opt_hd_min_rows.load(std::memory_order_relaxed);
        const int hd_shape = (int)g_opt_hd_shape.load(std::memory_order_relaxed);
        const bool hd = NB <= 3 && ((hd_mask >> (NB - 1)) & 1) && a.n_out >= hd_min_rows;
        if (hd || !(a.splits > 1 && !a.perm_per_split && (long long)grid.x * grid.y <= CV_SPLIT_TICKETS)) a.tickets = nullptr;
        if (hd) {
            const int nw = hd_shape == 1 ? 4 : 8;
            launch_conv_hd(a, NB, hd_shape, ma, dim3((unsigned)((a.n_out + nw * 32 - 1) / (nw * 32)), grid.y, grid.z), st);
        } else {
            launch_conv_hl(a, NB, ma, grid, st);
        }
    } else if (vec && a.wp6 && per_wg <= WP_NPRE) {
        launch_conv_rows_wp(a, NB, a.pieces, false, grid, st);
    } else if (vec && a.wp6 && per_wg <= WP_NPRE_BIG) {
        launch_conv_rows_wp(a, NB, a.pieces, true, grid, st);
    } else {
        CV_REQUIRE(a.pieces != 1 || !(vec && a.wp6), CV_EINVAL, "the bf16 compute mode takes at most %d kernel offsets per workgroup", WP_NPRE_BIG);
        CV_REQUIRE(!a.in2, CV_EINVAL,
                   "a second source takes at most %d kernel offsets per workgroup (%d here: flavour 0 with a workspace splits the "
                   "launch, or pass fewer offsets per call)", WP_NPRE_BIG, per_wg);
        launch_conv_rows(a, NB, vec, grid, st);
    }
    CV_LAUNCH_CHECK();
    return a.splits > 1 && !a.tickets ? launch_finish(a, st, ma, models) : CV_OK;
}

int nb_for(int cout) {
    static const int nb_max = getenv("CV_NB_MAX") ? atoi(getenv("CV_NB_MAX")) : 0;
    if (nb_max > 0) return std::min(nb_max, nb_full(cout));
    if (cout <= 32) return 1;
    if (cout <= 64) return 2;
    if (cout <= 96) return 3;
    static const int nb_wide = getenv("CV_NB_WIDE") ? atoi(getenv("CV_NB_WIDE")) : 2;
    return std::max(1, std::min(nb_wide, 2));
}

std::atomic<long long> g_split_target{-1};
thread_local long long t_split_target = 0;
long long process_split_target() {
    long long v = g_split_target.load(std::memory_order_relaxed);
    if (v <= 0) {
        v = getenv("CV_SPLIT_TARGET") ? std::max(1ll, atoll(getenv("CV_SPLIT_TARGET"))) : 768;
        g_split_target.store(v, std::memory_order_relaxed);
    }
    return v;
}
long long split_target() { return t_split_target > 0 ? t_split_target : process_split_target(); }

int pick_splits(long long n_out, int cout, int K, int cin, bool vec) {
    const int nb = nb_for(cout);
    const long long tiles = ((n_out + TM - 1) / TM) * ((cout + nb * 32 - 1) / (nb * 32));
    const long long units = vec ? (long long)K * (cin / KC) : ((long long)K * cin + KC - 1) / KC;
    if (tiles >= 384 || units <= 1) return 1;
    const long long target = split_target();
    long long s = (target + tiles - 1) / tiles;
    s = std::min(s, units);
    static const long long traffic_mb = getenv("CV_SPLIT_TRAFFIC_MB") ? atoll(getenv("CV_SPLIT_TRAFFIC_MB")) : 24;
    const long long by_traffic = (traffic_mb << 20) / std::max<long long>(1, n_out * cout * 4);
    s = std::min(s, std::max<long long>(by_traffic, 2));
    s = std::min<long long>(s, 64);
    return (int)std::max<long long>(s, 1);
}

}

static std::atomic<long long>* option_named(const char* name) {
    return !strcmp(name, "hd_mask") ? &g_opt_hd_mask : !strcmp(name, "hd_min_rows") ? &g_opt_hd_min_rows :
           !strcmp(name, "hd_shape") ? &g_opt_hd_shape : !strcmp(name, "zskip") ? &g_opt_zskip :
           !strcmp(name, "zskip_launches") ? &g_zskip_launches : nullptr;
}

int cv_sp_set_option(const char* name, long long value, long long* previous) {
    CV_REQUIRE(name, CV_EINVAL, "null option name");
    std::atomic<long long>* o = option_named(name);
    CV_REQUIRE(o, CV_EINVAL, "unknown option '%s' (hd_mask, hd_min_rows, hd_shape, zskip, zskip_launches)", name);
    const long long before = o->exchange(value, std::memory_order_relaxed);
    if (previous) *previous = before;
    return CV_OK;
}

int cv_sp_get_option(const char* name, long long* value) {
    CV_REQUIRE(name && value, CV_EINVAL, "null option name / value");
    const std::atomic<long long>* o = option_named(name);
    CV_REQUIRE(o, CV_EINVAL, "unknown option '%s'", name);
    *value = o->load(std::memory_order_relaxed);
    return CV_OK;
}

int cv_sp_set_ablation(int bits) { return g_ablation.exchange(bits, std::memory_order_relaxed); }

int cv_sp_set_split_target_thread(int workgroups) {
    const int before = (int)t_split_target;
    t_split_target = workgroups > 0 ? workgroups : 0;
    return before;
}

int cv_sp_set_split_target(int workgroups) {
    const int before = (int)process_split_target();
    g_split_target.store(workgroups > 0 ? workgroups : -1, std::memory_order_relaxed);
    return before;
}

static int conv_dispatch(const cv_conv_desc* d, const CvConvModels* mm, void* stream);

extern "C" {

size_t cv_sp_conv_workspace_bytes(long long n_out, int cout, int K) {
    if (n_out <= 0 || cout <= 0 || K <= 0) return 0;
    const size_t one = sizeof(float) * (size_t)n_out * (size_t)cout;
    return 256 + std::min<size_t>(64 * one, std::max<size_t>((size_t)48 << 20, 3 * one));
}

int cv_sp_conv_f32(const cv_conv_desc* d, void* stream) { return conv_dispatch(d, nullptr, stream); }

}

int cv_sp_conv_models_f32(const cv_conv_desc* d, const CvConvModels* mm, void* stream) {
    CV_REQUIRE(d && mm && mm->d_params && mm->models >= 1 && mm->models <= CV_MAX_CATEGORIES, CV_EINVAL, "bad model-axis arguments");
    CV_REQUIRE(!d->split_tickets, CV_EINVAL, "the model axis does not take split_tickets");
    CV_REQUIRE(d->weight_pieces == 2 && !d->acc_in && !d->acc_scale_dev, CV_EINVAL,
               "the model axis runs fp16-pair programs only (weight_pieces == 2; no bf16 triples, no fp32 convolution)");
    CV_REQUIRE(((mm->in_stride | mm->in2_stride | mm->res_stride | mm->out_stride | mm->ws_stride) & 127) == 0, CV_EINVAL,
               "model strides must keep rows 128-byte aligned");
    return conv_dispatch(d, mm, stream);
}

static int conv_dispatch(const cv_conv_desc* d, const CvConvModels* mm, void* stream) {
    CV_REQUIRE(d, CV_EINVAL, "null descriptor");
    CV_REQUIRE(d->in && d->weight && d->out, CV_EINVAL, "null pointer argument");
    CV_REQUIRE(d->n_in > 0 && d->n_out > 0 && d->cin > 0 && d->cout > 0 && d->K > 0, CV_EINVAL, "bad conv sizes");
    CV_REQUIRE(d->nbr || (d->K == 1 && d->n_in == d->n_out), CV_EINVAL, "a kernel map is required unless K == 1");
    CV_REQUIRE(d->in_ld >= d->cin && d->out_ld >= d->cout && (!d->residual || d->res_ld >= d->cout) &&
                   (!d->acc_in || d->acc_ld >= d->cout), CV_EINVAL, "bad leading dimension");
    CV_REQUIRE(d->out != d->in, CV_EINVAL, "conv cannot run in place");
    const int jb = d->j_begin, je = d->j_end > 0 ? d->j_end : d->K;
    CV_REQUIRE(jb >= 0 && jb < je && je <= d->K, CV_EINVAL, "bad kernel offset range");
    hipStream_t st = static_cast<hipStream_t>(stream);
    ConvArgs a = {};
    a.in = d->in, a.n_in = d->n_in, a.in_ld = d->in_ld, a.cin = d->cin;
    a.w = d->weight, a.K = d->K, a.cout = d->cout;
    a.nbr = d->nbr, a.n_out = d->n_out;
    a.scale = d->scale, a.shift = d->shift;
    a.res = d->residual, a.res_ld = d->res_ld;
    a.relu = d->relu;
    a.out = d->out, a.out_ld = d->out_ld;
    a.splits = 1;
    a.row_perm = d->row_perm;
    a.j_begin = jb, a.j_end = je;
    a.acc_in = d->acc_in, a.acc_ld = d->acc_ld;
    a.wp6 = static_cast<const unsigned short*>(d->weight_x6);
    a.in2 = d->in2, a.in2_ld = d->in2_ld, a.cin2 = d->cin2;
    a.wp6_2 = static_cast<const unsigned short*>(d->weight2_x6);
    a.pieces = d->weight_pieces == 2 ? 2 : d->weight_pieces == 1 ? 1 : 3;
    a.acc_scale = d->acc_scale != 0.f ? d->acc_scale : 1.f;
    a.range_flag = d->range_flag;
    a.in_hl = d->in_hl, a.out_hl = d->out_hl, a.res_hl = d->res_hl;
    a.tickets = d->in_hl ? d->split_tickets : nullptr;
    if (d->in_hl || d->out_hl || d->res_hl) {
        CV_REQUIRE(!d->in_hl || (d->weight_pieces == 2 && d->cin % 32 == 0 && d->in_ld % 32 == 0 &&
                                 (reinterpret_cast<uintptr_t>(d->in) & 127) == 0 &&
                                 (!d->in2 || (d->cin2 % 32 == 0 && d->in2_ld % 32 == 0 &&
                                              (reinterpret_cast<uintptr_t>(d->in2) & 127) == 0))),
                   CV_EINVAL, "hl-format input: fp16-pair weights, channels and leading dimensions %% 32 == 0, 128-byte aligned rows");
        CV_REQUIRE(!d->out_hl || (d->cout % 32 == 0 && d->out_ld % 32 == 0 && (reinterpret_cast<uintptr_t>(d->out) & 127) == 0),
                   CV_EINVAL, "hl-format output: Cout and leading dimension %% 32 == 0, 128-byte aligned rows");
        CV_REQUIRE(!d->res_hl || !d->residual || (d->res_ld % 32 == 0 && (reinterpret_cast<uintptr_t>(d->residual) & 127) == 0),
                   CV_EINVAL, "hl-format residual: leading dimension %% 32 == 0, 128-byte aligned rows");
        CV_REQUIRE(d->flavour == 0, CV_EINVAL, "the hl format runs with flavour 0 only");
        CV_REQUIRE(!d->in_hl || ((unsigned long long)d->n_in * (unsigned long long)d->in_ld * 4ull + (unsigned long long)d->cin * 4ull < (1ull << 32) &&
                                 (!d->in2 || (unsigned long long)d->n_out * (unsigned long long)d->in2_ld * 4ull + (unsigned long long)d->cin2 * 4ull < (1ull << 32))),
                   CV_EINVAL, "hl-format input larger than 4 GiB (rows x leading dimension x 4): split the batch");
    }
    CV_REQUIRE(d->weight_pieces >= 0 && d->weight_pieces <= 3, CV_EINVAL,
               "weight_pieces is 0/3 (bf16 triples), 2 (fp16 pairs) or 1 (single bf16 product)");
    CV_REQUIRE(d->weight_pieces != 1 || (d->weight_x6 && d->cin % KC == 0), CV_EINVAL,
               "weight_pieces = 1 needs weight_x6 from cv_sp_pack_weights_bf16_f32 and Cin %% 32 == 0");
    const bool stem_h2 = d->weight_pieces == 2 && d->weight_x6 && d->cout == 32 && (d->cin == 3 || d->cin == 6) && d->K <= 128;
    CV_REQUIRE(d->weight_pieces != 2 || stem_h2 || (d->weight_x6 && d->cin % KC == 0), CV_EINVAL,
               "weight_pieces = 2 needs weight_x6 from cv_sp_pack_weights_h2_f32 and Cin %% 32 == 0 (or the stem shape with "
               "cv_sp_pack_weights_stem_h2_f32)");

    ModelArgs ma = {};
    if (mm) {
        ma.params = mm->d_params;
        ma.in_stride = mm->in_stride, ma.in2_stride = mm->in2_stride, ma.res_stride = mm->res_stride, ma.out_stride = mm->out_stride;
        ma.partial_stride = mm->ws_stride;
        ma.out_ext = mm->out_ext;
        for (int m = 0; m < mm->models; ++m) ma.ext_out[m] = mm->ext_out[m];
    }
    ModelArgs* const pma = mm ? &ma : nullptr;
    const int models = mm ? mm->models : 1;
    CV_REQUIRE(!d->plan_ent && !d->plan_cnt && !d->weight_packed && (d->flavour == 0 || d->flavour == 1), CV_EINVAL,
               "flavours 3 / 4 (the experimental wave / tile kernels of rounds 1-3) are gone: flavour is 0 or 1, plan_ent / plan_cnt / "
               "weight_packed must be NULL");
    a.wide = d->cout % 4 == 0 && d->out_ld % 4 == 0 && (!d->residual || d->res_ld % 4 == 0) &&
             (!d->acc_in || d->acc_ld % 4 == 0) &&
             ((reinterpret_cast<uintptr_t>(d->out) | reinterpret_cast<uintptr_t>(d->residual) |
               reinterpret_cast<uintptr_t>(d->acc_in) | reinterpret_cast<uintptr_t>(d->scale) |
               reinterpret_cast<uintptr_t>(d->shift) | reinterpret_cast<uintptr_t>(d->ws)) & 15) == 0;
    CV_REQUIRE(a.wide || (!d->out_hl && !d->res_hl), CV_EINVAL,
               "hl-format output / residual: Cout, leading dimensions %% 4 == 0 and 16-byte aligned out, residual, acc_in, "
               "scale, shift and ws");
    const bool vec = (d->cin % KC == 0) && (d->in_ld % 4 == 0) && (d->cout % 4 == 0) &&
                     ((reinterpret_cast<uintptr_t>(d->in) & 15) == 0) &&
                     ((reinterpret_cast<uintptr_t>(d->weight) & 15) == 0);
    CV_REQUIRE(!d->weight_x6 || vec || stem_h2, CV_EINVAL,
               "weight_x6 needs the vector path: Cin %% 32 == 0, Cout %% 4 == 0, in_ld %% 4 == 0, 16-byte aligned in / weight");
    if (d->in2) {
        CV_REQUIRE(vec && d->weight_x6 && d->weight2_x6 && d->cin2 > 0 && d->cin2 % KC == 0 && d->in2_ld >= d->cin2 &&
                       d->in2_ld % 4 == 0 && (reinterpret_cast<uintptr_t>(d->in2) & 15) == 0,
                   CV_EINVAL, "a second source needs the bf16x6 vector path (weight_x6, weight2_x6, Cin2 %% 32 == 0, "
                              "16-byte aligned rows)");
    }
    if (!vec && d->cout == 32 && (d->cin == 3 || d->cin == 6) && d->nbr && !d->row_perm && d->perm_groups <= 1 &&
        d->flavour == 0) {
        if (d->weight_x6 && d->weight_pieces == 2 && d->K <= 128 && a.wide && !d->acc_in && d->j_begin == 0 &&
            (d->j_end == 0 || d->j_end == d->K)) {
            const dim3 g((unsigned)((d->n_out + TM - 1) / TM), (unsigned)models);
            if (d->cin == 3) with_models(pma, [&](auto... m) { conv_stem_mfma<3, decltype(m)...><<<g, THREADS, 0, st>>>(a, m...); });
            else with_models(pma, [&](auto... m) { conv_stem_mfma<6, decltype(m)...><<<g, THREADS, 0, st>>>(a, m...); });
            CV_LAUNCH_CHECK();
            return CV_OK;
        }
    }
    CV_REQUIRE(!mm || d->in_hl, CV_EINVAL, "the model axis runs fp16-pair programs on hl buffers only (and their matrix-core stem)");
    a.acc_scale_dev = d->acc_scale_dev;
    if (d->perm_groups > 1) {
        const size_t need = sizeof(float) * (size_t)d->perm_groups * (size_t)d->n_out * (size_t)d->cout;
        CV_REQUIRE(d->row_perm && vec && d->ws && d->ws_bytes >= need, CV_EINVAL,
                   "perm_groups needs row_perm[groups][n_out], Cin %% 32 == 0 and a workspace of %zu bytes", need);
        a.splits = d->perm_groups;
        a.perm_per_split = 1;
        a.partial = static_cast<float*>(d->ws);
        if (d->perm_has_map && jb == 0 && je == d->K && d->nbr) {
            a.nbr_perm = d->row_perm + (long long)d->perm_groups * d->n_out;
            a.nbr_perm_w = (d->K + d->perm_groups - 1) / d->perm_groups;
            if (g_opt_zskip.load(std::memory_order_relaxed) && d->valid_words && d->K <= 32 && !d->in2 && a.wide &&
                d->perm_groups <= FINISH_SMALL_MAX && d->in_hl) {
                a.gvalid = d->valid_words;
                g_zskip_launches.fetch_add(1, std::memory_order_relaxed);
            }
        }
    } else if (d->flavour == 0) {
        int sp = pick_splits(d->n_out, d->cout, je - jb, d->cin, vec);
        if (d->in_hl || (vec && a.wp6)) {
            const int nj = je - jb;
            const int per_wg = sp <= 1 ? nj : (nj + sp - 1) / sp + 1;
            if (per_wg > WP_NPRE) sp = std::max(sp, (nj + WP_NPRE - 2) / (WP_NPRE - 1));
        }
        const size_t need = sizeof(float) * (size_t)sp * (size_t)d->n_out * (size_t)d->cout;
        CV_REQUIRE(!d->in_hl || sp <= 1 || (d->ws && d->ws_bytes >= need), CV_ENOMEM,
                   "hl-format convolution needs a workspace of %zu bytes (cv_sp_conv_workspace_bytes)", need);
        if (sp > 1 && d->ws && d->ws_bytes >= need) {
            a.splits = sp;
            a.partial = static_cast<float*>(d->ws);
        }
    }
    return launch_rows(a, nb_for(d->cout), vec, st, pma, models);
}
```

canonicalvoting_amd/csrc/sparse_conv_common.h:

```cpp
#pragma once
#include "cv_common.h"

#include <type_traits>
#include <utility>

namespace cvsc {

typedef float f32x16 __attribute__((ext_vector_type(16)));

constexpr int KC = 32;
constexpr int TM = 128;
constexpr int A_LD = TM + 2;
constexpr int THREADS = 256;

#ifndef CV_WP_NPRE
#define CV_WP_NPRE 10
#endif
constexpr int WP_NPRE = CV_WP_NPRE;
constexpr int WP_NPRE_BIG = 28;
constexpr int HL_MAX_UNITS = 512;

struct ConvArgs {
    const float* in; long long n_in; int in_ld; int cin;
    const float* w; int K; int cout;
    const int* nbr; long long n_out;
    const float* scale; const float* shift;
    const float* res; int res_ld;
    int relu;
    float* out; int out_ld;
    int splits;
    float* partial;
    const int* row_perm;
    int perm_per_split;
    int j_begin, j_end;
    const float* acc_in;
    int acc_ld;
    int wide;
    const int* nbr_perm;
    int nbr_perm_w;
    const unsigned short* wp6;
    const float* in2;
    int in2_ld, cin2;
    const unsigned short* wp6_2;
    int pieces;
    float acc_scale;
    int* range_flag;
    int in_hl, out_hl, res_hl;
    int* tickets;
    const float* acc_scale_dev;
    const int* gvalid;
};

struct ModelArgs {
    const cv_net_model_params* params;
    long long in_stride, in2_stride, res_stride, out_stride, partial_stride;
    int ncb;
    int out_ext;
    float* ext_out[CV_MAX_CATEGORIES];
};
template <class T>
__device__ __forceinline__ T* model_offset(T* p, long long bytes) {
    return p ? reinterpret_cast<T*>(reinterpret_cast<uintptr_t>(p) + (uintptr_t)bytes) : p;
}
__device__ __forceinline__ void model_sources(ConvArgs& a, const ModelArgs& ma, int m) {
    const cv_net_model_params& p = ma.params[m];
    a.in = model_offset(a.in, m * ma.in_stride);
    a.in2 = model_offset(a.in2, m * ma.in2_stride);
    a.wp6 = static_cast<const unsigned short*>(p.weight_x6);
    a.wp6_2 = static_cast<const unsigned short*>(p.weight2_x6);
}
__device__ __forceinline__ void model_sinks(ConvArgs& a, const ModelArgs& ma, int m) {
    const cv_net_model_params& p = ma.params[m];
    a.res = model_offset(a.res, m * ma.res_stride);
    a.out = ma.out_ext ? ma.ext_out[m] : model_offset(a.out, m * ma.out_stride);
    a.partial = model_offset(a.partial, m * ma.partial_stride);
    a.range_flag = a.range_flag ? a.range_flag + 16 * m : nullptr;
    a.scale = p.scale;
    a.shift = p.shift;
    a.acc_scale = p.acc_scale;
}
__device__ __forceinline__ unsigned model_enter(ConvArgs&, unsigned by) { return by; }
__device__ __forceinline__ unsigned model_enter(ConvArgs& a, unsigned by, const ModelArgs& ma) {
    const unsigned m = by / (unsigned)ma.ncb;
    model_sources(a, ma, (int)m);
    return by - m * (unsigned)ma.ncb;
}
__device__ __forceinline__ void model_epilogue(ConvArgs&, unsigned) {}
__device__ __forceinline__ void model_epilogue(ConvArgs& a, unsigned by_grid, const ModelArgs& ma) {
    model_sinks(a, ma, (int)(by_grid / (unsigned)ma.ncb));
}
__device__ __forceinline__ void model_enter_y(ConvArgs&) {}
__device__ __forceinline__ void model_enter_y(ConvArgs& a, const ModelArgs& ma) {
    model_sources(a, ma, (int)blockIdx.y);
    model_sinks(a, ma, (int)blockIdx.y);
}

template <class F>
void with_models(const ModelArgs* ma, F&& f) {
    if (ma) f(*ma);
    else f();
}
template <int MAX, class F>
void with_nb(int nb, F&& f) {
    if constexpr (MAX > 1) {
        if (nb < MAX) return with_nb<MAX - 1>(nb, f);
    }
    f(std::integral_constant<int, MAX>{});
}

__device__ __forceinline__ long long tile_of(const ConvArgs& a) {
    return a.row_perm ? (long long)gridDim.x - 1 - blockIdx.x : blockIdx.x;
}

void launch_conv_rows(const ConvArgs& a, int nb, bool vec, dim3 grid, hipStream_t st);
void launch_conv_rows_wp(const ConvArgs& a, int nb, int pieces, bool npre_big, dim3 grid, hipStream_t st);
void launch_conv_hl(const ConvArgs& a, int nb, const ModelArgs* ma, dim3 grid, hipStream_t st);
void launch_conv_hd(const ConvArgs& a, int nb, int hd_shape, const ModelArgs* ma, dim3 grid, hipStream_t st);

__device__ __forceinline__ void hl_split2(float x0, float x1, unsigned& h, unsigned& l);
__device__ __forceinline__ float4 hl_load4(const float* row, int col) {
    const unsigned char* p = reinterpret_cast<const unsigned char*>(row) + (col >> 5) * 128 + (col & 31) * 2;
    const uint2 h = *reinterpret_cast<const uint2*>(p), l = *reinterpret_cast<const uint2*>(p + 64);
    typedef _Float16 h2 __attribute__((ext_vector_type(2)));
    const h2 h0 = __builtin_bit_cast(h2, h.x), h1 = __builtin_bit_cast(h2, h.y), l0 = __builtin_bit_cast(h2, l.x),
             l1 = __builtin_bit_cast(h2, l.y);
    return make_float4((float)h0[0] + (float)l0[0], (float)h0[1] + (float)l0[1], (float)h1[0] + (float)l1[0],
                       (float)h1[1] + (float)l1[1]);
}
__device__ __forceinline__ void hl_store4(float* row, int col, float4 v) {
    unsigned h0, l0, h1, l1;
    hl_split2(v.x, v.y, h0, l0);
    hl_split2(v.z, v.w, h1, l1);
    unsigned char* p = reinterpret_cast<unsigned char*>(row) + (col >> 5) * 128 + (col & 31) * 2;
    *reinterpret_cast<uint2*>(p) = make_uint2(h0, h1);
    *reinterpret_cast<uint2*>(p + 64) = make_uint2(l0, l1);
}
__device__ __forceinline__ bool hl_out_of_range(float4 v) {
    return fmaxf(fmaxf(fabsf(v.x), fabsf(v.y)), fmaxf(fabsf(v.z), fabsf(v.w))) > 65000.f;
}

typedef float f32x4v __attribute__((ext_vector_type(4)));
__device__ __forceinline__ void partial_store4(float* p, float4 v) {
    f32x4v t; t[0] = v.x; t[1] = v.y; t[2] = v.z; t[3] = v.w;
    __builtin_nontemporal_store(t, reinterpret_cast<f32x4v*>(p));
}
__device__ __forceinline__ void partial_store4_wt(float* p, float4 v) {
    f32x4v t; t[0] = v.x; t[1] = v.y; t[2] = v.z; t[3] = v.w;
    asm volatile("global_store_dwordx4 %0, %1, off sc1\n\ts_nop 1" :: "v"(p), "v"(t) : "memory");
}
__device__ __forceinline__ float4 partial_load4(const float4* p) {
    const f32x4v t = __builtin_nontemporal_load(reinterpret_cast<const f32x4v*>(p));
    return make_float4(t[0], t[1], t[2], t[3]);
}

__device__ __forceinline__ void epilogue_apply1(const ConvArgs& a, long long row, int col, float v, float sc, float sh) {
    if (a.acc_in) v += a.acc_in[row * a.acc_ld + col];
    v = v * sc + sh;
    if (a.res) v += a.res[row * a.res_ld + col];
    if (a.relu) v = fmaxf(v, 0.f);
    a.out[row * a.out_ld + col] = v;
}
__device__ __forceinline__ void epilogue_apply1(const ConvArgs& a, long long row, int col, float v) {
    epilogue_apply1(a, row, col, v, a.scale ? a.scale[col] : 1.f, a.shift ? a.shift[col] : 0.f);
}

__device__ __forceinline__ __attribute__((used)) void epilogue_store(const ConvArgs& a, const f32x16& acc, const int* rows,
                                               int col, int lane) {
    if (col >= a.cout) return;
    if (a.splits > 1) {
        float* p = a.partial + (long long)blockIdx.z * a.n_out * a.cout;
#pragma unroll
        for (int r = 0; r < 16; ++r) {
            const int row = rows[(r & 3) + 8 * (r >> 2) + 4 * (lane >> 5)];
            if (row >= 0) p[(long long)row * a.cout + col] = acc[r];
        }
        return;
    }
    const float sc = a.scale ? a.scale[col] : 1.f;
    const float sh = a.shift ? a.shift[col] : 0.f;
#pragma unroll
    for (int r = 0; r < 16; ++r) {
        const int row = rows[(r & 3) + 8 * (r >> 2) + 4 * (lane >> 5)];
        if (row >= 0) epilogue_apply1(a, row, col, acc[r], sc, sh);
    }
}

__device__ __forceinline__ void epilogue_apply4(const ConvArgs& a, long long row, int col, float4 v) {
    if (a.acc_in) {
        const float4 p = *reinterpret_cast<const float4*>(a.acc_in + row * a.acc_ld + col);
        v.x += p.x; v.y += p.y; v.z += p.z; v.w += p.w;
    }
    const float4 sc = a.scale ? *reinterpret_cast<const float4*>(a.scale + col) : make_float4(1.f, 1.f, 1.f, 1.f);
    const float4 sh = a.shift ? *reinterpret_cast<const float4*>(a.shift + col) : make_float4(0.f, 0.f, 0.f, 0.f);
    v.x = v.x * sc.x + sh.x; v.y = v.y * sc.y + sh.y; v.z = v.z * sc.z + sh.z; v.w = v.w * sc.w + sh.w;
    if (a.res) {
        const float4 p = a.res_hl ? hl_load4(a.res + row * a.res_ld, col)
                                  : *reinterpret_cast<const float4*>(a.res + row * a.res_ld + col);
        v.x += p.x; v.y += p.y; v.z += p.z; v.w += p.w;
    }
    if (a.relu) { v.x = fmaxf(v.x, 0.f); v.y = fmaxf(v.y, 0.f); v.z = fmaxf(v.z, 0.f); v.w = fmaxf(v.w, 0.f); }
    if (a.out_hl) {
        if (a.range_flag && hl_out_of_range(v)) *a.range_flag = 1;
        hl_store4(a.out + row * a.out_ld, col, v);
    } else {
        *reinterpret_cast<float4*>(a.out + row * a.out_ld + col) = v;
    }
}

constexpr int EP_LD = 36;
__device__ __forceinline__ __attribute__((used)) void epilogue_store_wide(const ConvArgs& a, const f32x16& acc, const int* rows, int colbase,
                                                    int lane, float (*T)[EP_LD]) {
    const int h = lane >> 5, c = lane & 31;
#pragma unroll
    for (int r = 0; r < 16; ++r) T[(r & 3) + 8 * (r >> 2) + 4 * h][c] = acc[r];
    __builtin_amdgcn_fence(__ATOMIC_RELEASE, "wavefront");
    __builtin_amdgcn_wave_barrier();
    __builtin_amdgcn_fence(__ATOMIC_ACQUIRE, "wavefront");
    const int col = colbase + (lane & 7) * 4;
    if (col < a.cout) {
#pragma unroll
        for (int it = 0; it < 4; ++it) {
            const int rl = (lane >> 3) + 8 * it;
            const int row = rows[rl];
            if (row < 0) continue;
            float4 v = *reinterpret_cast<const float4*>(&T[rl][(lane & 7) * 4]);
            if (a.splits > 1) {
                float* pp = a.partial + ((long long)blockIdx.z * a.n_out + row) * a.cout + col;
                if (a.tickets) partial_store4_wt(pp, v);
                else partial_store4(pp, v);
                continue;
            }
            epilogue_apply4(a, row, col, v);
        }
    }
    __builtin_amdgcn_wave_barrier();
}

typedef short bf16x8 __attribute__((ext_vector_type(8)));

typedef __bf16 bf16x2v __attribute__((ext_vector_type(2)));
typedef float f32x2v __attribute__((ext_vector_type(2)));
__device__ __forceinline__ unsigned cvt_pk_bf16(float lo, float hi) {
    const f32x2v v = {lo, hi};
    return __builtin_bit_cast(unsigned, __builtin_convertvector(v, bf16x2v));
}
__device__ __forceinline__ void split3(float x0, float x1, unsigned& h, unsigned& m, unsigned& l) {
    h = cvt_pk_bf16(x0, x1);
    const float r0 = x0 - __uint_as_float(h << 16), r1 = x1 - __uint_as_float(h & 0xffff0000u);
    m = cvt_pk_bf16(r0, r1);
    const float s0 = r0 - __uint_as_float(m << 16), s1 = r1 - __uint_as_float(m & 0xffff0000u);
    l = cvt_pk_bf16(s0, s1);
}

typedef _Float16 f16x2 __attribute__((ext_vector_type(2)));
typedef _Float16 f16x8 __attribute__((ext_vector_type(8)));
__device__ __forceinline__ void split2h(float x0, float x1, unsigned& h, unsigned& l) {
    const f16x2 hv = {(_Float16)x0, (_Float16)x1};
    h = __builtin_bit_cast(unsigned, hv);
    float r0, r1;
    asm("v_fma_mix_f32 %0, %1, -1.0, %2 op_sel_hi:[1,0,0]" : "=v"(r0) : "v"(h), "v"(x0));
    asm("v_fma_mix_f32 %0, %1, -1.0, %2 op_sel:[1,0,0] op_sel_hi:[1,0,0]" : "=v"(r1) : "v"(h), "v"(x1));
    const f16x2 lv = {(_Float16)r0, (_Float16)r1};
    l = __builtin_bit_cast(unsigned, lv);
}

__device__ __forceinline__ void hl_split2(float x0, float x1, unsigned& h, unsigned& l) { split2h(x0, x1, h, l); }

__device__ __forceinline__ float sum_in_order4(const float* __restrict__ p, int n, long long stride) {
    float s0 = 0.f, s1 = 0.f, s2 = 0.f, s3 = 0.f;
    int k = 0;
    for (; k + 3 < n; k += 4) {
        s0 += p[k * stride];
        s1 += p[(k + 1) * stride];
        s2 += p[(k + 2) * stride];
        s3 += p[(k + 3) * stride];
    }
    for (; k < n; ++k) s0 += p[k * stride];
    return (s0 + s1) + (s2 + s3);
}

template <int... I, class F>
__device__ __forceinline__ void static_for_impl(std::integer_sequence<int, I...>, F&& f) {
    (f(std::integral_constant<int, I>{}), ...);
}
template <int N, class F>
__device__ __forceinline__ void static_for(F&& f) { static_for_impl(std::make_integer_sequence<int, N>{}, f); }

static __device__ __attribute__((aligned(128))) unsigned char g_zero_chunk[128];
template <int N>
__device__ __forceinline__ void wait_vmcnt_le() { asm volatile("s_waitcnt vmcnt(%0)" :: "n"(N) : "memory"); }
__device__ __forceinline__ void wait_vmcnt_dyn(int n) {
    switch (n) {
        case 0: wait_vmcnt_le<0>(); break;
        case 1: wait_vmcnt_le<1>(); break;
        case 2: wait_vmcnt_le<2>(); break;
        case 3: wait_vmcnt_le<3>(); break;
        case 4: wait_vmcnt_le<4>(); break;
        case 5: wait_vmcnt_le<5>(); break;
        case 6: wait_vmcnt_le<6>(); break;
        case 7: wait_vmcnt_le<7>(); break;
        default: wait_vmcnt_le<8>(); break;
    }
}
typedef __attribute__((address_space(3))) void* lds_ptr_t;
__device__ __forceinline__ void lds_dma16(const void* g, unsigned char* l) {
    __builtin_amdgcn_global_load_lds(g, (lds_ptr_t)l, 16, 0, 0);
}
typedef unsigned u32x4v __attribute__((ext_vector_type(4)));
template <int NB>
__device__ __forceinline__ void hd_read_frags(unsigned aa0, unsigned aa1, unsigned ab, u32x4v& A0, u32x4v& A1,
                                              u32x4v (&B0)[NB], u32x4v (&B1)[NB]) {
    constexpr int P1 = NB * 32 * 64;
    if constexpr (NB == 1) {
        asm volatile("ds_read_b128 %0, %4\n\tds_read_b128 %1, %5\n\tds_read_b128 %2, %6\n\tds_read_b128 %3, %6 offset:%7\n\t"
                     "s_waitcnt lgkmcnt(0)"
                     : "=&v"(A0), "=&v"(A1), "=&v"(B0[0]), "=&v"(B1[0])
                     : "v"(aa0), "v"(aa1), "v"(ab), "i"(P1) : "memory");
    } else if constexpr (NB == 2) {
        asm volatile("ds_read_b128 %0, %6\n\tds_read_b128 %1, %7\n\tds_read_b128 %2, %8\n\tds_read_b128 %3, %8 offset:%9\n\t"
                     "ds_read_b128 %4, %8 offset:%10\n\tds_read_b128 %5, %8 offset:%11\n\t"
                     "s_waitcnt lgkmcnt(0)"
                     : "=&v"(A0), "=&v"(A1), "=&v"(B0[0]), "=&v"(B1[0]), "=&v"(B0[1]), "=&v"(B1[1])
                     : "v"(aa0), "v"(aa1), "v"(ab), "i"(P1), "i"(2048), "i"(P1 + 2048) : "memory");
    } else {
        static_assert(NB == 3, "conv_hd: 32, 64 or 96 columns per workgroup");
        asm volatile("ds_read_b128 %0, %8\n\tds_read_b128 %1, %9\n\tds_read_b128 %2, %10\n\tds_read_b128 %3, %10 offset:%11\n\t"
                     "ds_read_b128 %4, %10 offset:%12\n\tds_read_b128 %5, %10 offset:%13\n\t"
                     "ds_read_b128 %6, %10 offset:%14\n\tds_read_b128 %7, %10 offset:%15\n\t"
                     "s_waitcnt lgkmcnt(0)"
                     : "=&v"(A0), "=&v"(A1), "=&v"(B0[0]), "=&v"(B1[0]), "=&v"(B0[1]), "=&v"(B1[1]), "=&v"(B0[2]), "=&v"(B1[2])
                     : "v"(aa0), "v"(aa1), "v"(ab), "i"(P1), "i"(2048), "i"(P1 + 2048), "i"(4096), "i"(P1 + 4096) : "memory");
    }
}

inline int nb_full(int cout) { return cout <= 32 ? 1 : cout <= 64 ? 2 : cout <= 96 ? 3 : 4; }
__host__ inline bool aligned16(const void* p) { return (reinterpret_cast<uintptr_t>(p) & 15) == 0; }
}
```

canonicalvoting_amd/me/__init__.py:

```python
import ctypes
import math
import os
import threading
import weakref

import numpy as np
import torch
import torch.nn as nn

from .. import _lib
from .._lib import ptr as _ptr, stream as _stream, vp
from . import utils

__version__ = "0.5.3-cvhip"


class _NoSwitch:
    def __enter__(self):
        return self

    def __exit__(self, *exc):
        return False


# ... 203 lines not shown
            out_map = ibuf[o_inv:o_inv + n].view(n, 1)
            for i in range(4):
                cm_s._maps[("k", 2, 1 << i, 2)] = view(off.down[i], c[i + 1], 8)
                cm_s._maps[("up", 16 >> i)] = view(off.up[i], c[3 - i], 8)
                cm_s._maps[("upperm", 16 >> i)] = arena[off.up_perm[i]:off.up_perm[i] + c[3 - i]]
            for i in range(5):
                cm_s._maps[("k", 3, 1 << i, 1)] = view(off.k3[i], c[i], 27)
                if i == 0 or off.mask_perm[i] >= 0:
                    cm_s._maps[("k", 3, 1 << i, 1)]._cv_valid_words = arena[off.k3[i] + 27 * c[i]:off.k3[i] + 28 * c[i]]
                if off.mask_perm[i] >= 0:
                    mp = view(off.mask_perm[i], G, c[i])
                    mp._cv_has_map = True
                    mp._cv_from_plan = True
                    cm_s._maps[("mp", 3, 1 << i, G)] = mp
                    cm_s._maps[("k", 3, 1 << i, 1)]._cv_mask_perms = mp
            plan.views = (cm_s, stem_map, out_map)
        return plan.views

    def num_rows(self, ts):
        if ts == 1:
            return self._input.shape[0]
        if ts not in self._level:
            self.ensure_levels()
        return self.counts[self._level[ts]]

    def kernel_map(self, k, ts_in, stride=1):
        if ts_in * stride not in self._level:
            self.ensure_levels()
        self._verify()
        key = ("k", k, ts_in, stride)
        m = self._maps.get(key)
        if m is None:
            L = _lib.lib()
            li = self._level[ts_in]
            out = self.coords[ts_in * stride]
            m = torch.empty((out.shape[0], k ** 3), dtype=torch.int32, device=self.device)
            with torch.cuda.device(self.device):
                _lib.check(L.cv_sp_kernel_map(_ptr(out), out.shape[0], _ptr(self._keys[li]),
                                              _ptr(self._vals[li]), self.cap, k, ts_in, _ptr(m),
                                              _stream(self.device)), "cv_sp_kernel_map")
            self._maps[key] = m
        return m

    def up_map(self, ts_coarse):
        key = ("up", ts_coarse)
        m = self._maps.get(key)
        if m is None:
            L = _lib.lib()
            down = self.kernel_map(2, ts_coarse // 2, 2)
            n_fine = self.num_rows(ts_coarse // 2)
            m = torch.empty((n_fine, 8), dtype=torch.int32, device=self.device)
            with torch.cuda.device(self.device):
                _lib.check(L.cv_sp_up_map(_ptr(down), down.shape[0], n_fine, _ptr(m), _stream(self.device)),
                           "cv_sp_up_map")
            self._maps[key] = m
        return m


class SparseTensor:

    def __init__(self, features, coordinates=None, device=None, coordinate_manager=None, tensor_stride=1,
                 **_):
        if device is None:
            device = features.device if coordinates is None else (
                features.device if features.is_cuda else torch.device("cuda"))
        device = torch.device(device)
        if device.type != "cuda":
            raise RuntimeError("canonicalvoting_amd SparseTensor runs on the GPU only (no CPU engine); "
                               "pass device='cuda'")
        self.F = features.to(device=device, dtype=torch.float32)
        self.F_hl = None
        if coordinate_manager is None:
            if coordinates is None:
                raise ValueError("coordinates or coordinate_manager required")
            c = coordinates
            if c.is_floating_point():
                c = torch.floor(c)
            coordinate_manager = CoordinateManager(c.to(device=device, dtype=torch.int32).contiguous(),
                                                   num_levels=1, check=False, lazy=True)
        self.coordinate_manager = coordinate_manager
        self.tensor_stride = tensor_stride if isinstance(tensor_stride, int) else int(tensor_stride[0])
        if self.F.shape[0] != coordinate_manager.num_rows(self.tensor_stride):
            raise RuntimeError("features have %d rows, coordinate set has %d" % (
                self.F.shape[0], coordinate_manager.num_rows(self.tensor_stride)))

    @property
    def C(self):
        cm = self.coordinate_manager
        if self.tensor_stride not in cm.coords:
            cm.ensure_levels()
        return cm.coords[self.tensor_stride]

    @property
    def coordinates(self):
        return self.C

    @property
    def features(self):
        return self.F

    @property
    def device(self):
        return self.F.device

    @property
    def shape(self):
        return self.F.shape

    def __len__(self):
        return self.F.shape[0]

    @property
    def decomposed_coordinates_and_features(self):
        C, Fm = self.C, self.F
        nb = int(C[:, 0].max().item()) + 1
        cs, fs = [], []
        for b in range(nb):
            m = C[:, 0] == b
            cs.append(C[m][:, 1:])
            fs.append(Fm[m])
        return cs, fs

    def _like(self, F, tensor_stride=None, F_hl=None):
        t = SparseTensor(F, coordinate_manager=self.coordinate_manager,
                         tensor_stride=self.tensor_stride if tensor_stride is None else tensor_stride)
        t.F_hl = F_hl
        return t


def _workspace(dev, nbytes):
    return _lib.scratch(dev, "conv_ws", nbytes)


_range_flags = {}
_range_lock = threading.Lock()


def range_flag(dev):
    key = (dev, torch.cuda.current_stream(dev).cuda_stream)
    with _range_lock:
        f = _range_flags.get(key)
        if f is None:
            f = _range_flags[key] = torch.zeros(1, dtype=torch.int32).pin_memory()
    return f


def _piece_path(cin, cout, flavour=0):
    return CONV_X6 and flavour in (0, 1) and cin % 32 == 0 and cout % 4 == 0


def conv_forward(x_feats, weight, nbr, n_out, scale=None, shift=None, residual=None, relu=False,
                 out=None, flavour=0, row_perm=None, j_begin=0, j_end=0, acc_in=None, perm_groups=0,
                 cache_weights=True, pieces=None, in_hl=False, out_hl=False, res_hl=False, stem_mfma=False,
                 split_tickets=None, weight_t=False, acc_scale_dev=None, step=None):
    if pieces is None:
        pieces = 1 if COMPUTE_DTYPE == "bf16" else 3
    L = _lib.lib()
    dev = x_feats.device
    w = weight if weight.dim() == 3 else weight[None]
    if weight_t and not _piece_path(w.shape[2], w.shape[1], flavour):
        w, weight_t = w.permute(0, 2, 1), False
    w = w.contiguous()
    K, cin, cout = (w.shape[0], w.shape[2], w.shape[1]) if weight_t else w.shape
    assert x_feats.shape[1] == cin and x_feats.stride(1) == 1
    if out is None:
        out = torch.empty((n_out, cout), dtype=torch.float32, device=dev)
    if (AUTO_MASK_GROUPS > 1 and row_perm is None and perm_groups == 0 and flavour == 0 and nbr is not None
            and K == 27 and n_out >= AUTO_MASK_MIN_ROWS and cin % 32 == 0 and j_begin == 0 and j_end == 0
            and acc_in is None):
        row_perm = map_mask_perms(nbr, AUTO_MASK_GROUPS)
        perm_groups = row_perm.shape[0]
    wp, _, weight_pieces, acc_scale, folded = resolve_weights(
        weight, w, pieces, flavour=flavour, transposed=weight_t, stem=stem_mfma and nbr is not None and flavour == 0,
        col_scale=scale, cache=cache_weights, step=step if step is not None else current_step())
    if folded:
        scale = None
    ws = None
    if perm_groups > 1:
        ws = _workspace(dev, 4 * perm_groups * n_out * cout + 256)
    elif flavour == 0 and n_out < 128 * 384:
        ws = _workspace(dev, int(L.cv_sp_conv_workspace_bytes(n_out, cout, K)))
    d = _lib.ConvDesc(in_=x_feats.data_ptr(), n_in=x_feats.shape[0], in_ld=x_feats.stride(0), cin=cin, weight=w.data_ptr(),
                      K=K, cout=cout, n_out=n_out, relu=bool(relu), out=out.data_ptr(), out_ld=out.stride(0), flavour=flavour,
                      perm_groups=perm_groups, weight_pieces=weight_pieces, acc_scale=acc_scale, in_hl=bool(in_hl),
                      out_hl=bool(out_hl), res_hl=bool(res_hl))
    if nbr is not None:
        d.nbr = nbr.data_ptr()
    if scale is not None:
        d.scale = scale.data_ptr()
    if shift is not None:
        d.shift = shift.data_ptr()
    if residual is not None:
        d.residual, d.res_ld = residual.data_ptr(), residual.stride(0)
    if ws is not None:
        d.ws, d.ws_bytes = ws.data_ptr(), ws.numel()
    if row_perm is not None:
        d.row_perm, d.perm_has_map = row_perm.data_ptr(), bool(perm_groups > 1 and getattr(row_perm, "_cv_has_map", False))
        if d.perm_has_map and nbr is not None and K <= 32 and option("zskip"):
            d.valid_words = map_valid_words(nbr).data_ptr()
    if j_begin or j_end:
        d.j_begin, d.j_end = j_begin, j_end
    if acc_in is not None:
        d.acc_in, d.acc_ld = acc_in.data_ptr(), acc_in.stride(0)
    if wp is not None:
        d.weight_x6 = wp.data_ptr()
    if weight_pieces == 2:
        d.range_flag = range_flag(dev).data_ptr()
    if split_tickets is not None:
        d.split_tickets = split_tickets.data_ptr()
    if acc_scale_dev is not None:
        d.acc_scale_dev = acc_scale_dev.data_ptr()
    with _on(dev):
        _lib.check(L.cv_sp_conv_f32(ctypes.byref(d), _stream(dev)), "cv_sp_conv_f32")
    return out


_policy_tls = threading.local()


def masked_min_rows():
    v = getattr(_policy_tls, "masked_min_rows", None)
    return CoordinateManager.MASKED_MIN_ROWS if v is None else v


def set_masked_min_rows_thread(rows):
    before = getattr(_policy_tls, "masked_min_rows", None)
    _policy_tls.masked_min_rows = None if rows is None else int(rows)
    return before


def set_split_target(workgroups):
    return int(_lib.lib().cv_sp_set_split_target(int(workgroups)))


def set_option(name, value):
    prev = ctypes.c_longlong(0)
    _lib.check(_lib.lib().cv_sp_set_option(name.encode(), int(value), ctypes.byref(prev)), "cv_sp_set_option")
    return int(prev.value)


def option(name):
    v = ctypes.c_longlong(0)
    _lib.check(_lib.lib().cv_sp_get_option(name.encode(), ctypes.byref(v)), "cv_sp_get_option")
    return int(v.value)


def to_hl(x):
    y = torch.empty((x.shape[0], x.shape[1]), dtype=torch.float32, device=x.device)
    with _on(x.device):
        _lib.check(_lib.lib().cv_sp_to_hl_f32(x.data_ptr(), x.shape[0], x.shape[1], x.stride(0), y.data_ptr(), y.stride(0),
                                              range_flag(x.device).data_ptr(), _stream(x.device)), "cv_sp_to_hl_f32")
    return y


def from_hl(x):
    y = torch.empty((x.shape[0], x.shape[1]), dtype=torch.float32, device=x.device)
    with _on(x.device):
        _lib.check(_lib.lib().cv_sp_from_hl_f32(x.data_ptr(), x.shape[0], x.shape[1], x.stride(0), y.data_ptr(),
                                                y.stride(0), _stream(x.device)), "cv_sp_from_hl_f32")
    return y


AUTO_MASK_GROUPS = int(os.environ.get("CV_MASK_GROUPS", "4"))
AUTO_MASK_MIN_ROWS = int(os.environ.get("CV_AUTO_MASK_MIN_ROWS", "16384"))


def map_mask_perms(nbr, groups):
    hit = getattr(nbr, "_cv_mask_perms", None)
    if hit is not None and getattr(hit, "_cv_from_plan", False):
        return hit
    if hit is None or hit.shape[0] != groups:
        hit = nbr._cv_mask_perms = _perms_with_map(nbr, groups)
    return hit


def map_valid_words(nbr):
    hit = getattr(nbr, "_cv_valid_words", None)
    if hit is None:
        bits = torch.ones(nbr.shape[1], dtype=torch.int64, device=nbr.device) << torch.arange(nbr.shape[1], device=nbr.device)
        hit = nbr._cv_valid_words = ((nbr >= 0) * bits).sum(1).to(torch.int32)
    return hit


def _perms_with_map(nbr, groups):
    L = _lib.lib()
    n, K = nbr.shape
    W = (K + groups - 1) // groups
    flat = torch.empty(groups * n * (1 + W) + (groups * n + 3) // 4, dtype=torch.int32, device=nbr.device)
    ws = torch.empty(groups * 4096, dtype=torch.uint8, device=nbr.device)
    with _on(nbr.device):
        _lib.check(L.cv_sp_mask_perms(_ptr(nbr), n, K, groups, _ptr(flat), _ptr(ws), ws.numel(), 1,
                                      _stream(nbr.device)), "cv_sp_mask_perms")
    m = flat[:groups * n].view(groups, n)
    m._cv_has_map = True
    m._cv_flat = flat
    return m


CONV_X6 = os.environ.get("CV_CONV_X6", "1") != "0"


COMPUTE_DTYPE = "bf16" if os.environ.get("CV_COMPUTE_DTYPE", "fp32") == "bf16" else "fp32"


def set_compute_dtype(dtype):
    global COMPUTE_DTYPE
    assert dtype in ("fp32", "bf16"), dtype
    prev, COMPUTE_DTYPE = COMPUTE_DTYPE, dtype
    return prev


def pack_weights(w3, pieces, col_scale=None, scale_log2=0, transposed=False, stem=False):
    L = _lib.lib()
    dev = w3.device
    K, c1, c2 = w3.shape
    assert not (transposed and col_scale is not None) and not (stem and (pieces != 2 or c2 != 32))
    wp = torch.empty(8 * c1 * 1024 if stem else pieces * w3.numel(), dtype=torch.int16, device=dev)
    args, k, st = (_ptr(w3), K, c1, c2), int(scale_log2), _stream(dev)
    with _on(dev):
        if stem:
            _lib.check(L.cv_sp_pack_weights_stem_h2_f32(_ptr(w3), K, c1, _ptr(col_scale), k, _ptr(wp), st),
                       "cv_sp_pack_weights_stem_h2_f32")
        elif transposed:
            _lib.check(L.cv_sp_pack_weights_t_f32(*args, pieces, k, _ptr(wp), st), "cv_sp_pack_weights_t_f32")
        elif pieces == 2:
            _lib.check(L.cv_sp_pack_weights_h2_f32(*args, _ptr(col_scale), k, _ptr(wp), st), "cv_sp_pack_weights_h2_f32")
        elif pieces == 1:
            _lib.check(L.cv_sp_pack_weights_bf16_f32(*args, _ptr(col_scale), _ptr(wp), st), "cv_sp_pack_weights_bf16_f32")
        else:
            _lib.check(L.cv_sp_pack_weights_x6_f32(*args, _ptr(col_scale), _ptr(wp), st), "cv_sp_pack_weights_x6_f32")
    return wp


def h2_scale_log2(*scaled_weights):
    amax = 0.0
    for w3, col_scale in scaled_weights:
        a = w3.abs().amax(dim=(0, 1)) if col_scale is not None else w3.abs().max()
        amax = max(amax, float((a * col_scale.abs()).max()) if col_scale is not None else float(a))
    if not math.isfinite(amax) or amax <= 0.0:
        return 0
    return max(-60, min(60, 13 - math.ceil(math.log2(amax))))


_pack_cache = {}


def invalidate_weight_caches():
    _pack_cache.clear()


def _cached_packings(weight):
    key = id(weight)
    ver = (weight.data_ptr(), weight._version, tuple(weight.shape))
    hit = _pack_cache.get(key)
    if hit is None or hit[1] != ver or hit[0]() is not weight:
        hit = _pack_cache[key] = (weakref.ref(weight, lambda _r, k=key: _pack_cache.pop(k, None)), ver, {})
    return hit[2]


def resolve_weights(weight, w3, pieces, flavour=0, transposed=False, stem=False, col_scale=None, second=None, cache=False,
                    step=None):
    K, cin, cout = (w3.shape[0], w3.shape[2], w3.shape[1]) if transposed else w3.shape
    stem = stem and pieces == 2 and cin in (3, 6) and cout == 32 and K <= 128
    if not stem and not _piece_path(cin, cout, flavour):
# ... 663 lines not shown
```

include/cv_hip.h:

```cpp
#ifndef CV_HIP_H
#define CV_HIP_H

#include <stddef.h>
#include <stdint.h>

#ifdef __cplusplus
extern "C" {
#endif

#define CV_OK 0
#define CV_EINVAL (-22)
#define CV_ENOMEM (-12)
#define CV_EHIP (-5)
#define CV_ERANGE (-34)

#define CV_ABI_VERSION 6
int cv_abi_version(void);
const char* cv_last_error(void);


size_t cv_hv_minmax_workspace_bytes(void);
int cv_hv_minmax_f32(const float* d_points, int64_t n, float* h_min3, float* h_max3,
                     void* d_ws, size_t ws_bytes, void* stream);
int cv_hv_minmax_async_f32(const float* d_points, int64_t n, float* h_minmax6, void* d_ws, size_t ws_bytes,
// ... 103 lines not shown
                       int32_t* const* d_vals, long long n, long long cap, int num_levels,
                       int32_t* d_counts, int32_t* h_counts, void* d_ws, size_t ws_bytes, void* stream);

#define CV_QUANTIZE_MAX_CLOUDS 256
size_t cv_sp_quantize_workspace_bytes(long long m);
int cv_sp_quantize_f32(const float* d_points, long long m, long long ld, float quantization_size, int floor_only,
                       const long long* h_offsets, int n_clouds, int32_t* d_coords4, int32_t* d_index, int32_t* d_inverse,
                       int32_t* d_counts, int32_t* h_counts, void* d_ws, size_t ws_bytes, void* stream);
int cv_sp_quantize_f64(const double* d_points, long long m, long long ld, double quantization_size, int floor_only,
                       const long long* h_offsets, int n_clouds, int32_t* d_coords4, int32_t* d_index, int32_t* d_inverse,
                       int32_t* d_counts, int32_t* h_counts, void* d_ws, size_t ws_bytes, void* stream);

#define CV_GATHER_MAX_JOBS 8
typedef struct cv_gather_job {
    const void* d_src; long long src_ld;
    void* d_dst; long long dst_ld;
    int width;
    int recentre_from;
} cv_gather_job;
int cv_sp_voxel_rows_f32(const int32_t* d_coords4, const int32_t* d_index, long long n, float res, float* d_points_out,
                         const cv_gather_job* jobs, int n_jobs, void* stream);

typedef struct cv_scan_rows_desc {
    const int32_t* d_coords4; const int32_t* d_index; long long n;
    long long m_points;
    const float* d_points; long long points_ld;
    const uint8_t* d_rgb;
    const int32_t* d_owner;
    const double* d_minv; const float* d_model_scale; const int32_t* d_model_cls; int n_models;
    const double* d_colour; const double* d_jitter; int n_clouds;
    int use_xyz, recentre;
    float* d_feats; long long feats_ld;
    float* d_xyz; long long xyz_ld;
    float* d_scale; long long scale_ld;
    long long* d_cls; long long cls_ld;
} cv_scan_rows_desc;
int cv_sp_scan_rows_f32(const cv_scan_rows_desc* desc, void* stream);

typedef struct cv_sym_loss_desc {
    const float* d_out; long long n_rows; long long ld;
    const int32_t* d_rows; const int32_t* d_pseg; long long n_points;
    const int32_t* d_seg_ptr; const int32_t* d_pose_ptr; const int32_t* d_tgt_ptr; int n_segments; int n_jobs;
    const float* d_targets; long long n_targets;
    const int32_t* d_urow; const int32_t* d_uptr; const int32_t* d_upoint; int n_urows;
    float w[3]; float xyz_factor;
    float* d_loss; float* d_pose_loss; int32_t* d_best; float* d_seg_loss;
    const float* d_grad_loss; float* d_grad; long long grad_ld;
    void* d_ws; size_t ws_bytes;
} cv_sym_loss_desc;
int cv_sym_loss_fwd_f32(const cv_sym_loss_desc* desc, void* stream);
int cv_sym_loss_bwd_f32(const cv_sym_loss_desc* desc, void* stream);
size_t cv_sym_loss_workspace_bytes(long long n_targets, int n_jobs);
int cv_sym_loss_chunk_rows(void);

#define CV_ROW_LOSS_GATHER_LABEL 0
#define CV_ROW_LOSS_GATHER_ARGMAX 1
#define CV_ROW_LOSS_EMPTY_ZERO 0
#define CV_ROW_LOSS_EMPTY_NAN 1
typedef struct cv_row_loss_desc {
    const float* d_out; long long n_rows; long long ld;
    const int64_t* d_labels;
    const float* d_xyz_labels; const float* d_scale_labels;
    int heads; int n_logits; int xyz_col; int scale_col; int logit_col;
    long long obj_lo; long long obj_hi;
    int with_xyz; int log_scale; int gather; int empty;
    float w[3]; float xyz_factor; float scale_factor;
    float* d_losses; int32_t* d_info;
    const float* d_grad_loss; float* d_grad; long long grad_ld; int n_cols;
    void* d_ws; size_t ws_bytes;
} cv_row_loss_desc;
int cv_row_loss_fwd_f32(const cv_row_loss_desc* desc, void* stream);
int cv_row_loss_bwd_f32(const cv_row_loss_desc* desc, void* stream);
size_t cv_row_loss_workspace_bytes(long long n_rows);
int cv_row_loss_chunk_rows(void);

typedef struct cv_sym_rows_desc {
    const int32_t* d_coords4; const int32_t* d_index; const int32_t* d_inverse;
    const int32_t* d_quant_counts;
    long long m_points;
    const float* d_points; long long points_ld;
    const uint8_t* d_rgb;
    const int32_t* d_owner;
    const float* d_model_scale; const int32_t* d_model_cls; int n_models;
    const double* d_colour; const double* d_jitter;
    const long long* d_offsets; int n_clouds;
    const int32_t* d_seg_vertex; long long n_cand;
    const int32_t* d_seg_vptr; const int32_t* d_seg_pose_ptr; int n_seg_in;
    const double* d_minv; long long n_jobs_in;
    long long n_targets_in;
    int reference_indexing, use_xyz, recentre;
    int32_t* d_rows; int32_t* d_pseg; int32_t* d_seg_ptr; int32_t* d_pose_ptr; int32_t* d_tgt_ptr; float* d_targets;
    int32_t* d_urow; int32_t* d_uptr; int32_t* d_upoint;
    float* d_feats; long long feats_ld;
    float* d_scale; long long scale_ld;
    long long* d_obj; long long* d_cls;
    int32_t* d_counts; int32_t* h_counts;
    void* d_ws; size_t ws_bytes;
} cv_sym_rows_desc;
int cv_sp_sym_rows_f32(const cv_sym_rows_desc* desc, void* stream);
size_t cv_sp_sym_rows_workspace_bytes(long long m_points, long long n_cand, int n_seg_in, int n_clouds);
int cv_sp_sym_rows_block(void);
long long cv_sp_sym_rows_scan_span(void);

size_t cv_sp_sort_workspace_bytes(long long n);
int cv_sp_sort_rows(const int32_t* d_coords, long long n, int32_t* d_sorted, int32_t* d_perm, int32_t* d_inv,
                    void* d_ws, size_t ws_bytes, void* stream);

int cv_sp_morton_keys(const int32_t* d_coords, long long n, long long* d_keys, void* stream);

int cv_sp_kernel_map(const int32_t* d_out_coords, long long n_out, const unsigned long long* d_keys,
                     const int32_t* d_vals, long long cap, int k, int ts, int32_t* d_nbr, void* stream);

int cv_sp_up_map(const int32_t* d_nbr_down, long long n_coarse, long long n_fine, int32_t* d_up,
                 void* stream);

typedef struct cv_conv_desc {
    const float* in;
    long long n_in;
    int in_ld, cin;
    const float* weight;
    int K, cout;
    const int32_t* nbr;
    long long n_out;
    const float* scale;
    const float* shift;
    const float* residual;
    int res_ld;
    int relu;
    float* out;
    int out_ld;
    int flavour;
    void* ws;
    size_t ws_bytes;
    const int32_t* row_perm;
    int j_begin, j_end;
    const float* acc_in;
    int acc_ld;
    int perm_groups;
    const int32_t* plan_ent;
    const int32_t* plan_cnt;
    const float* weight_packed;
    const void* weight_x6;
    const float* in2;
    int in2_ld, cin2;
    const void* weight2_x6;
    int perm_has_map;
    int weight_pieces;
    float acc_scale;
    int32_t* range_flag;
    int in_hl, out_hl, res_hl;
    int32_t* split_tickets;
    const float* acc_scale_dev;
    const int32_t* valid_words;
} cv_conv_desc;
#define CV_SPLIT_TICKETS 4096

int cv_sp_to_hl_f32(const float* d_x, long long n, int c, int x_ld, float* d_y, int y_ld, int32_t* range_flag, void* stream);
int cv_sp_from_hl_f32(const float* d_x, long long n, int c, int x_ld, float* d_y, int y_ld, void* stream);

int cv_sp_pack_weights_x6_f32(const float* d_w, int K, int cin, int cout, const float* d_col_scale, void* d_wp6,
                              void* stream);
int cv_sp_pack_weights_h2_f32(const float* d_w, int K, int cin, int cout, const float* d_col_scale, int scale_log2,
                              void* d_wp, void* stream);
typedef struct cv_pack_job {
    const float* w;
    void* wp;
    int K, cin, cout;
    int trans;
    int scale_log2;
    int reserved;
} cv_pack_job;
int cv_sp_pack_weights_h2_batch_f32(const cv_pack_job* h_jobs, int n_jobs, void* d_jobs, void* stream);
int cv_sp_pack_weights_bf16_f32(const float* d_w, int K, int cin, int cout, const float* d_col_scale, void* d_wp,
                                void* stream);
int cv_sp_pack_weights_t_f32(const float* d_w, int K, int rows, int cols, int pieces, int scale_log2, void* d_wp, void* stream);
int cv_sp_pack_weights_stem_h2_f32(const float* d_w, int K, int cin, const float* d_col_scale, int scale_log2, void* d_wp,
                                   void* stream);

size_t cv_sp_conv_workspace_bytes(long long n_out, int cout, int K);
int cv_sp_conv_f32(const cv_conv_desc* desc, void* stream);

int cv_sp_set_split_target(int workgroups);
int cv_sp_set_split_target_thread(int workgroups);
int cv_sp_set_ablation(int bits);
int cv_sp_set_option(const char* name, long long value, long long* previous);
int cv_sp_get_option(const char* name, long long* value);

typedef struct cv_scene_maps {
    long long stem, out, down[4], k3[5], up[4], mask_perm[5], up_perm[4], scratch;
    long long bitmap;
} cv_scene_maps;
size_t cv_sp_scene_maps_words(const long long* level_rows, long long n_orig, int stem_k, int mask_groups,
                              long long masked_min_rows, cv_scene_maps* offsets);
int cv_sp_scene_maps(int32_t* const* d_coords, const unsigned long long* const* d_keys, const int32_t* const* d_vals,
                     long long cap, const long long* level_rows, const int32_t* d_perm, long long n_orig, int stem_k,
                     int mask_groups, long long masked_min_rows, int32_t* d_arena, size_t arena_words, void* stream);

size_t cv_sp_scene_plan_words(long long n, int stem_k, int mask_groups, long long masked_min_rows);
int cv_sp_scene_plan(const int32_t* d_input, long long n, int32_t* d_perm, int32_t* d_inv, int32_t* const* d_coords,
                     unsigned long long* const* d_keys, int32_t* const* d_vals, long long cap, int32_t* d_counts,
                     int32_t* h_counts, int stem_k, int mask_groups, long long masked_min_rows, int32_t* d_arena,
                     size_t arena_words, cv_scene_maps* offsets, void* d_sort_ws, size_t sort_ws_bytes, void* d_levels_ws,
                     size_t levels_ws_bytes, void* stream);

typedef struct cv_scene_plan_layout {
    long long cap;
    long long perm, inv, coords[5], vals[5], counts, arena;
    long long int_words, key_words;
    size_t sort_ws_bytes, levels_ws_bytes;
} cv_scene_plan_layout;
int cv_sp_scene_plan_layout(long long n, int stem_k, int mask_groups, long long masked_min_rows, cv_scene_plan_layout* out);
#define CV_NET_MAP_SLOTS 15
#define CV_NET_PERM_SLOTS 9
int cv_sp_scene_plan_slots(const cv_scene_plan_layout* layout, const cv_scene_maps* offsets, const long long* level_rows,
                           long long min_rows, const int32_t* d_ibuf, const int32_t** maps, const int32_t** perms);
size_t cv_sp_scene_conv_workspace_bytes(const long long* level_rows, const int* masked, int mask_groups, int max_channels);

typedef struct cv_net_buf {
    int level, channels, rows_level;
    int hl;
} cv_net_buf;
typedef struct cv_net_op {
    int in_buf, in_col, cin;
    int out_buf, out_col, cout;
    int res_buf, res_col;
    int map, K;
    int perm, perm_groups;
    int relu;
    const float* weight;
    const float* scale;
    const float* shift;
    const void* weight_x6;
    int in2_buf, in2_col, cin2;
    const void* weight2_x6;
    int weight_pieces;
    float acc_scale;
} cv_net_op;
size_t cv_net_arena_bytes(const cv_net_buf* bufs, int n_bufs, const long long* level_rows, int n_levels);
int cv_net_run_f32(const cv_net_op* ops, int n_ops, const cv_net_buf* bufs, int n_bufs, const long long* level_rows,
                   int n_levels, void* d_arena, size_t arena_bytes, const void* const* ext_ptr, const int* ext_ld,
                   const int32_t* const* maps, int n_maps, const int32_t* const* perms, int n_perms,
                   void* d_ws, size_t ws_bytes, int32_t* range_flag, void* stream);

typedef struct cv_net_model_params {
    const void* weight_x6;
    const void* weight2_x6;
    const float* scale;
    const float* shift;
    float acc_scale;
    int reserved[3];
} cv_net_model_params;
size_t cv_net_models_params_bytes(int n_ops, int K);
int cv_net_models_params_fill(const cv_net_op* const* ops, int n_ops, int K, void* h_params, size_t params_bytes);
size_t cv_net_models_arena_bytes(const cv_net_buf* bufs, int n_bufs, const long long* level_rows, int n_levels, int K);
size_t cv_net_models_workspace_bytes(size_t one_model_bytes, int K);
int cv_net_run_models_f32(const cv_net_op* const* ops, const cv_net_buf* const* bufs, int n_ops, int n_bufs, int K,
                          const long long* level_rows, int n_levels, void* d_arena, size_t arena_bytes,
                          const void* const* const* ext_ptr, const int* ext_ld, const int32_t* const* maps, int n_maps,
                          const int32_t* const* perms, int n_perms, void* d_ws, size_t ws_bytes, int32_t* range_flag,
                          const void* d_params, int params_ld, void* stream);

int cv_sp_mask_keys(const int32_t* d_nbr, long long n, int K, int j_begin, int j_end, long long* d_keys,
                    void* stream);

int cv_sp_mask_perms(const int32_t* d_nbr, long long n, int K, int groups, int32_t* d_perm, void* d_ws,
                     size_t ws_bytes, int with_map, void* stream);

int cv_sp_transpose_map(const int32_t* d_nbr, long long n_out, int K, long long n_in, int32_t* d_nbr_t, void* stream);
size_t cv_sp_wgrad_workspace_bytes(long long n_out, int cin, int cout, int K);
int cv_sp_conv_wgrad_f32(const float* d_x, int x_ld, int cin, const float* d_dy, int dy_ld, int cout,
                         const int32_t* d_nbr, int K, long long n_out, float* d_dw, void* d_ws, size_t ws_bytes,
                         void* stream);
int cv_sp_conv_wgrad_px_f32(const float* d_x, int x_ld, int cin, const float* d_dy, int dy_ld, int cout,
                            const int32_t* d_nbr, int K, long long n_out, float* d_dw, void* d_ws, size_t ws_bytes,
                            int pieces, void* stream);
int cv_sp_col_sum_f32(const float* d_x, long long n, int c, int ld, float* d_out, void* stream);
size_t cv_sp_col_sum_workspace_bytes(long long n, int c);
int cv_sp_col_sum_det_f32(const float* d_x, long long n, int c, int ld, float* d_out, void* d_ws, size_t ws_bytes,
                          void* stream);

size_t cv_sp_bn_workspace_bytes(int c);
int cv_sp_bn_stats_f32(const float* d_x, long long n, int c, int ld, const float* d_gamma, const float* d_beta,
                       float eps, float momentum, float* d_running_mean, float* d_running_var, float* d_mean,
                       float* d_var, float* d_scale, float* d_shift, void* d_ws, size_t ws_bytes, void* stream);
int cv_sp_bn_backward_f32(const float* d_x, const float* d_dy, const float* d_y, long long n, int c, int ld,
                          const float* d_mean, const float* d_var, float eps, const float* d_gamma, float* d_dgamma,
                          float* d_dbeta, float* d_dx, float* d_dres, void* d_ws, size_t ws_bytes, void* stream);

#define CV_BN_SLOT_WORDS 8200
int cv_sp_bn_backward_hl_f32(const float* d_x, const float* d_dy, const float* d_y, long long n, int c, int ld,
                             const float* d_mean, const float* d_var, float eps, const float* d_gamma, float* d_dgamma,
                             float* d_dbeta, float* d_dx, float* d_dres, void* d_ws, size_t ws_bytes, float* d_dx_hl,
                             uint32_t* d_slot, int32_t* range_flag, const uint32_t* d_relu_bits, void* stream);

int cv_sp_copy_unless_flag(const void* const* h_src, void* const* h_dst, const long long* h_bytes, int n, const int32_t* flag,
                           void* stream);

int cv_sp_affine_f32(const float* d_x, long long n, int c, int x_ld, const float* d_scale,
                     const float* d_shift, const float* d_residual, int res_ld, int relu, float* d_y, int y_ld,
                     void* stream);
int cv_sp_affine_hl_f32(const float* d_x, long long n, int c, int x_ld, const float* d_scale, const float* d_shift,
                        const float* d_residual, int res_ld, int relu, float* d_y, int y_ld, float* d_y_hl, int y_hl_ld,
                        uint32_t* d_relu_bits, int32_t* range_flag, void* stream);

int cv_sp_bn_fold_f32(const float* d_gamma, const float* d_beta, const float* d_mean, const float* d_var,
                      const float* d_bias, float eps, int c, float* d_scale, float* d_shift, void* stream);
// ... 181 lines not shown
```

Measured before the change: 695.1.

## Finish split-K group reduction inside the last group's conv kernel

Adds a group_finish mode for mask-permuted split convolutions. The other groups write partials, then a final launch with a fixed group runs its own slice and sums the other groups' partials, masked per row by valid words, straight in the epilogue. This removes the separate reduction pass or ticket-based last-block reduce. It adds a second launch, templated FIN kernel variants, and nontemporal partial loads, and it depends on launch ordering between the groups.

Measured after the change: 693.3. No clear change (-0.3%).

```diff
diff --git a/canonicalvoting_amd/_lib.py b/canonicalvoting_amd/_lib.py
--- a/canonicalvoting_amd/_lib.py
+++ b/canonicalvoting_amd/_lib.py
@@ -35,7 +35,8 @@
                 ("weight_packed", vp), ("weight_x6", vp), ("in2", vp), ("in2_ld", ctypes.c_int), ("cin2", ctypes.c_int),
                 ("weight2_x6", vp), ("perm_has_map", ctypes.c_int), ("weight_pieces", ctypes.c_int),
                 ("acc_scale", ctypes.c_float), ("range_flag", vp), ("in_hl", ctypes.c_int), ("out_hl", ctypes.c_int),
-                ("res_hl", ctypes.c_int), ("split_tickets", vp), ("acc_scale_dev", vp), ("valid_words", vp)]
+                ("res_hl", ctypes.c_int), ("split_tickets", vp), ("acc_scale_dev", vp), ("valid_words", vp),
+                ("group_finish", ctypes.c_int)]
 
 
 class SceneMaps(ctypes.Structure):
diff --git a/canonicalvoting_amd/csrc/conv_hd.hip b/canonicalvoting_amd/csrc/conv_hd.hip
--- a/canonicalvoting_amd/csrc/conv_hd.hip
+++ b/canonicalvoting_amd/csrc/conv_hd.hip
@@ -15,9 +15,10 @@
     const int b = (160 * 1024) / hd_lds_bytes(NB, NW, NSTG);
     return b * NW > 32 ? 32 / NW : (b < 1 ? 1 : b);
 }
-template <int NB, int NW, int NSTG, class... MA>
+template <int NB, int NW, int NSTG, bool FIN, class... MA>
 __global__ __launch_bounds__(NW * 64, (hd_blocks(NB, NW, NSTG) * NW + 3) / 4) void conv_hd(ConvArgs a, MA... ma) {
     const unsigned by = model_enter(a, blockIdx.y, ma...);
+    const int g = group_of<FIN>(a);
     static_assert(NSTG == 2 || NSTG == 3, "two or three ring stages");
     constexpr int TMv = NW * 32, THv = NW * 64;
     constexpr int A_BYTES = NW * 4096, B_BYTES = 2 * NB * 32 * 64, STAGE = A_BYTES + B_BYTES;
@@ -43,17 +44,17 @@
     const int nch = a.cin / KC;
     int u_lo, u_hi;
     if (a.perm_per_split) {
-        u_lo = (int)((long long)nj * blockIdx.z / a.splits) * nch;
-        u_hi = (int)((long long)nj * (blockIdx.z + 1) / a.splits) * nch;
+        u_lo = (int)((long long)nj * g / a.splits) * nch;
+        u_hi = (int)((long long)nj * (g + 1) / a.splits) * nch;
     } else {
-        u_lo = (int)((long long)nj * nch * blockIdx.z / a.splits);
-        u_hi = (int)((long long)nj * nch * (blockIdx.z + 1) / a.splits);
+        u_lo = (int)((long long)nj * nch * g / a.splits);
+        u_hi = (int)((long long)nj * nch * (g + 1) / a.splits);
     }
     const int j_first = a.j_begin + u_lo / nch, j_last = a.j_begin + (u_hi - 1) / nch;
     const int njl = u_hi > u_lo ? j_last - j_first + 1 : 0;
     const int nch2 = a.in2 ? a.cin2 / KC : 0;
 
-    const int* perm = a.row_perm ? a.row_perm + (a.perm_per_split ? (long long)blockIdx.z * a.n_out : 0) : nullptr;
+    const int* perm = a.row_perm ? a.row_perm + (a.perm_per_split ? (long long)g * a.n_out : 0) : nullptr;
     if (tid < TMv) {
         const long long t = tile_id * TMv + tid;
         const int row = t < a.n_out ? (perm ? perm[t] : (int)t) : -1;
@@ -62,14 +63,14 @@
     }
     {
         unsigned m = 0u;
-        const int jg0 = a.j_begin + (int)((long long)nj * blockIdx.z / a.splits);
+        const int jg0 = a.j_begin + (int)((long long)nj * g / a.splits);
         for (int e = tid; e < njl * TMv; e += THv) {
             const int jj = e / TMv, t = e - jj * TMv;
             const long long pos = tile_id * TMv + t;
             int v = -1;
             if (pos < a.n_out) {
                 if (a.nbr_perm) {
-                    v = a.nbr_perm[((long long)blockIdx.z * a.n_out + pos) * a.nbr_perm_w + (j_first + jj - jg0)];
+                    v = a.nbr_perm[((long long)g * a.n_out + pos) * a.nbr_perm_w + (j_first + jj - jg0)];
                 } else {
                     const int row = perm ? perm[pos] : (int)pos;
                     v = a.nbr ? a.nbr[(long long)row * a.K + j_first + jj] : row;
@@ -87,7 +88,7 @@
 #pragma unroll
     for (int w = 0; w < NW; ++w) lm |= wave_mask[w];
     if (wave == 0) {
-        const int n_first = u_hi - u_lo, n_second = nch2 > (int)blockIdx.z ? (nch2 - (int)blockIdx.z + a.splits - 1) / a.splits : 0;
+        const int n_first = u_hi - u_lo, n_second = nch2 > g ? (nch2 - g + a.splits - 1) / a.splits : 0;
         int cnt = 0;
         for (int base = 0; base < n_first + n_second; base += 64) {
             const int e = base + lane;
@@ -97,7 +98,7 @@
                 const int jj = a.j_begin + q - j_first;
                 if ((lm >> jj) & 1u) code = (jj << 8) | (u - q * nch);
             } else if (e < n_first + n_second) {
-                code = (njl << 8) | ((int)blockIdx.z + (e - n_first) * a.splits);
+                code = (njl << 8) | (g + (e - n_first) * a.splits);
             }
             const unsigned long long bal = __ballot(code >= 0);
             if (code >= 0) units_s[cnt + __popcll(bal & ((1ull << lane) - 1ull))] = (unsigned short)code;
@@ -107,7 +108,7 @@
     }
     __syncthreads();
     const int n_units = __builtin_amdgcn_readfirstlane((int)units_s[HL_MAX_UNITS]);
-    if (n_units == 0 && a.gvalid) return;
+    if (!FIN && n_units == 0 && a.gvalid) return;
 
     f32x16 acc[NB];
 #pragma unroll
@@ -252,7 +253,10 @@
     ConvArgs ae = a;
     ae.tickets = nullptr;
 #pragma unroll
-    for (int nb = 0; nb < NB; ++nb) epilogue_store_wide(ae, acc[nb], rows_s + wave * 32, n0 + nb * 32, lane, ep);
+    for (int nb = 0; nb < NB; ++nb) {
+        if constexpr (FIN) epilogue_finish_wide(ae, acc[nb], rows_s + wave * 32, n0 + nb * 32, lane, ep, g);
+        else epilogue_store_wide(ae, acc[nb], rows_s + wave * 32, n0 + nb * 32, lane, ep, g);
+    }
 }
 
 
@@ -261,8 +265,13 @@
 void cvsc::launch_conv_hd(const ConvArgs& a, int nb, int hd_shape, const ModelArgs* ma, dim3 grid, hipStream_t st) {
     with_nb<3>(nb, [&](auto nbc) {
         constexpr int NB = decltype(nbc)::value;
-        if (hd_shape == 1) with_models(ma, [&](auto... m) { conv_hd<NB, 4, 2, decltype(m)...><<<grid, 256, 0, st>>>(a, m...); });
-        else if (hd_shape == 2) with_models(ma, [&](auto... m) { conv_hd<NB, 8, 2, decltype(m)...><<<grid, 512, 0, st>>>(a, m...); });
-        else with_models(ma, [&](auto... m) { conv_hd<NB, 8, 3, decltype(m)...><<<grid, 512, 0, st>>>(a, m...); });
+        const auto with_fin = [&](auto fin) {
+            constexpr bool FIN = decltype(fin)::value;
+            if (hd_shape == 1) with_models(ma, [&](auto... m) { conv_hd<NB, 4, 2, FIN, decltype(m)...><<<grid, 256, 0, st>>>(a, m...); });
+            else if (hd_shape == 2) with_models(ma, [&](auto... m) { conv_hd<NB, 8, 2, FIN, decltype(m)...><<<grid, 512, 0, st>>>(a, m...); });
+            else with_models(ma, [&](auto... m) { conv_hd<NB, 8, 3, FIN, decltype(m)...><<<grid, 512, 0, st>>>(a, m...); });
+        };
+        if (a.group_fixed) with_fin(std::true_type{});
+        else with_fin(std::false_type{});
     });
 }
diff --git a/canonicalvoting_amd/csrc/conv_hl.hip b/canonicalvoting_amd/csrc/conv_hl.hip
--- a/canonicalvoting_amd/csrc/conv_hl.hip
+++ b/canonicalvoting_amd/csrc/conv_hl.hip
@@ -9,10 +9,11 @@
 namespace {
 
 constexpr int hl_blocks(int NB) { return NB <= 3 ? 4 : 2; }
-template <int NB, class... MA>
+template <int NB, bool FIN, class... MA>
 __global__ __attribute__((amdgpu_waves_per_eu(hl_blocks(NB), 8)))
 __launch_bounds__(THREADS, hl_blocks(NB)) void conv_hl(ConvArgs a, MA... ma) {
     const unsigned by = model_enter(a, blockIdx.y, ma...);
+    const int g = group_of<FIN>(a);
     constexpr int NS = 2, NW = THREADS / 64;
     constexpr int B_BYTES = 2 * NB * 32 * 64, EP_BYTES = NW * 32 * EP_LD * 4;
     constexpr int SM_BYTES = NS * B_BYTES > EP_BYTES ? NS * B_BYTES : EP_BYTES;
@@ -29,17 +30,17 @@
     const int nch = a.cin / KC;
     int u_lo, u_hi;
     if (a.perm_per_split) {
-        u_lo = (int)((long long)nj * blockIdx.z / a.splits) * nch;
-        u_hi = (int)((long long)nj * (blockIdx.z + 1) / a.splits) * nch;
+        u_lo = (int)((long long)nj * g / a.splits) * nch;
+        u_hi = (int)((long long)nj * (g + 1) / a.splits) * nch;
     } else {
-        u_lo = (int)((long long)nj * nch * blockIdx.z / a.splits);
-        u_hi = (int)((long long)nj * nch * (blockIdx.z + 1) / a.splits);
+        u_lo = (int)((long long)nj * nch * g / a.splits);
+        u_hi = (int)((long long)nj * nch * (g + 1) / a.splits);
     }
     const int j_first = a.j_begin + u_lo / nch, j_last = a.j_begin + (u_hi - 1) / nch;
     const int njl = u_hi > u_lo ? j_last - j_first + 1 : 0;
     const int nch2 = a.in2 ? a.cin2 / KC : 0;
 
-    const int* perm = a.row_perm ? a.row_perm + (a.perm_per_split ? (long long)blockIdx.z * a.n_out : 0) : nullptr;
+    const int* perm = a.row_perm ? a.row_perm + (a.perm_per_split ? (long long)g * a.n_out : 0) : nullptr;
     if (tid < TM) {
         const long long t = tile_id * TM + tid;
         const int row = t < a.n_out ? (perm ? perm[t] : (int)t) : -1;
@@ -48,14 +49,14 @@
     }
     {
         unsigned m = 0u;
-        const int jg0 = a.j_begin + (int)((long long)nj * blockIdx.z / a.splits);
+        const int jg0 = a.j_begin + (int)((long long)nj * g / a.splits);
         for (int e = tid; e < njl * TM; e += THREADS) {
             const int jj = e / TM, t = e - jj * TM;
             const long long pos = tile_id * TM + t;
             int v = -1;
             if (pos < a.n_out) {
                 if (a.nbr_perm) {
-                    v = a.nbr_perm[((long long)blockIdx.z * a.n_out + pos) * a.nbr_perm_w + (j_first + jj - jg0)];
+                    v = a.nbr_perm[((long long)g * a.n_out + pos) * a.nbr_perm_w + (j_first + jj - jg0)];
                 } else {
                     const int row = perm ? perm[pos] : (int)pos;
                     v = a.nbr ? a.nbr[(long long)row * a.K + j_first + jj] : row;
@@ -73,7 +74,7 @@
 #pragma unroll
     for (int w = 0; w < NW; ++w) lm |= wave_mask[w];
     if (wave == 0) {
-        const int n_first = u_hi - u_lo, n_second = nch2 > (int)blockIdx.z ? (nch2 - (int)blockIdx.z + a.splits - 1) / a.splits : 0;
+        const int n_first = u_hi - u_lo, n_second = nch2 > g ? (nch2 - g + a.splits - 1) / a.splits : 0;
         int cnt = 0;
         for (int base = 0; base < n_first + n_second; base += 64) {
             const int e = base + lane;
@@ -83,7 +84,7 @@
                 const int jj = a.j_begin + q - j_first;
                 if ((lm >> jj) & 1u) code = (jj << 8) | (u - q * nch);
             } else if (e < n_first + n_second) {
-                code = (njl << 8) | ((int)blockIdx.z + (e - n_first) * a.splits);
+                code = (njl << 8) | (g + (e - n_first) * a.splits);
             }
             const unsigned long long bal = __ballot(code >= 0);
             if (code >= 0) units_s[cnt + __popcll(bal & ((1ull << lane) - 1ull))] = (unsigned short)code;
@@ -93,7 +94,7 @@
     }
     __syncthreads();
     const int n_units = __builtin_amdgcn_readfirstlane((int)units_s[HL_MAX_UNITS]);
-    if (n_units == 0 && a.gvalid) return;
+    if (!FIN && n_units == 0 && a.gvalid) return;
 
     f32x16 acc[NB];
 #pragma unroll
@@ -118,6 +119,10 @@
     const unsigned char* const in_b = reinterpret_cast<const unsigned char*>(a.in);
     const unsigned char* const in2_b = reinterpret_cast<const unsigned char*>(a.in2);
 
+    typedef const __attribute__((address_space(1))) unsigned char* gbytes;
+    const auto gload16 = [](gbytes p) {
+        return __builtin_bit_cast(uint4, *reinterpret_cast<const __attribute__((address_space(1))) u32x4v*>(p));
+    };
     uint4 ra[NS][4], rb[NS][B_PER];
     bool live[NS];
 #pragma unroll
@@ -131,11 +136,17 @@
         live[sl] = __any(src >= 0);
         if (src >= 0) {
             const unsigned off = (unsigned)src * (second ? in2_row_bytes : in_row_bytes) + (unsigned)(c * 128 + half * 16);
-            const unsigned char* p = (second ? in2_b : in_b) + off;
-            ra[sl][0] = *reinterpret_cast<const uint4*>(p);
-            ra[sl][1] = *reinterpret_cast<const uint4*>(p + 32);
-            ra[sl][2] = *reinterpret_cast<const uint4*>(p + 64);
-            ra[sl][3] = *reinterpret_cast<const uint4*>(p + 96);
+            if constexpr (FIN && sizeof...(MA) > 0) {
+                const gbytes p = (gbytes)(second ? in2_b : in_b) + off;
+#pragma unroll
+                for (int q = 0; q < 4; ++q) ra[sl][q] = gload16(p + 32 * q);
+            } else {
+                const unsigned char* p = (second ? in2_b : in_b) + off;
+                ra[sl][0] = *reinterpret_cast<const uint4*>(p);
+                ra[sl][1] = *reinterpret_cast<const uint4*>(p + 32);
+                ra[sl][2] = *reinterpret_cast<const uint4*>(p + 64);
+                ra[sl][3] = *reinterpret_cast<const uint4*>(p + 96);
+            }
         } else {
 #pragma unroll
             for (int q = 0; q < 4; ++q) ra[sl][q] = make_uint4(0u, 0u, 0u, 0u);
@@ -143,8 +154,12 @@
         const unsigned short* slab = second ? a.wp6_2 + (size_t)c * slab_words
                                             : a.wp6 + (size_t)((j_first + jj) * nch + c) * slab_words;
 #pragma unroll
-        for (int i = 0; i < B_PER; ++i)
-            rb[sl][i] = b_src[i] >= 0 ? *reinterpret_cast<const uint4*>(slab + b_src[i]) : make_uint4(0u, 0u, 0u, 0u);
+        for (int i = 0; i < B_PER; ++i) {
+            if constexpr (FIN && sizeof...(MA) > 0)
+                rb[sl][i] = b_src[i] >= 0 ? gload16((gbytes)slab + 2u * (unsigned)b_src[i]) : make_uint4(0u, 0u, 0u, 0u);
+            else
+                rb[sl][i] = b_src[i] >= 0 ? *reinterpret_cast<const uint4*>(slab + b_src[i]) : make_uint4(0u, 0u, 0u, 0u);
+        }
     };
     auto stage_b = [&](auto S, int toff) {
         constexpr int sl = decltype(S)::value;
@@ -200,10 +215,15 @@
 #pragma unroll
             for (int r = 0; r < 16; ++r) acc[nb][r] *= sc;
     }
-    float (*ep)[EP_LD] = reinterpret_cast<float (*)[EP_LD]>(sm + wave * 32 * EP_LD * 4);
-#pragma unroll
-    for (int nb = 0; nb < NB; ++nb) epilogue_store_wide(a, acc[nb], rows_s + wave * 32, n0 + nb * 32, lane, ep);
-    if (a.splits > 1 && a.tickets) {
+    int lane_e = lane, wave_e = wave, g_e = g;
+    if constexpr (FIN) asm volatile("" : "+v"(lane_e), "+v"(wave_e), "+s"(g_e));
+    float (*ep)[EP_LD] = reinterpret_cast<float (*)[EP_LD]>(sm + wave_e * 32 * EP_LD * 4);
+#pragma unroll
+    for (int nb = 0; nb < NB; ++nb) {
+        if constexpr (FIN) epilogue_finish_wide<4>(a, acc[nb], rows_s + wave_e * 32, n0 + nb * 32, lane_e, ep, g_e);
+        else epilogue_store_wide(a, acc[nb], rows_s + wave_e * 32, n0 + nb * 32, lane_e, ep, g);
+    }
+    if constexpr (!FIN) if (a.splits > 1 && a.tickets) {
         __shared__ int last_flag;
         asm volatile("s_waitcnt vmcnt(0)" ::: "memory");
         __syncthreads();
@@ -250,6 +270,7 @@
 void cvsc::launch_conv_hl(const ConvArgs& a, int nb, const ModelArgs* ma, dim3 grid, hipStream_t st) {
     with_nb<4>(nb, [&](auto nbc) {
         constexpr int NB = decltype(nbc)::value;
-        with_models(ma, [&](auto... m) { conv_hl<NB, decltype(m)...><<<grid, THREADS, 0, st>>>(a, m...); });
+        if (a.group_fixed) with_models(ma, [&](auto... m) { conv_hl<NB, true, decltype(m)...><<<grid, THREADS, 0, st>>>(a, m...); });
+        else with_models(ma, [&](auto... m) { conv_hl<NB, false, decltype(m)...><<<grid, THREADS, 0, st>>>(a, m...); });
     });
 }
diff --git a/canonicalvoting_amd/csrc/conv_rows.hip b/canonicalvoting_amd/csrc/conv_rows.hip
--- a/canonicalvoting_amd/csrc/conv_rows.hip
+++ b/canonicalvoting_amd/csrc/conv_rows.hip
@@ -159,7 +159,7 @@
     if (a.wide) {
 #pragma unroll
         for (int nb = 0; nb < NB; ++nb)
-            epilogue_store_wide(a, acc[nb], rows_s + wave * 32, n0 + nb * 32, lane, ep_s[wave]);
+            epilogue_store_wide(a, acc[nb], rows_s + wave * 32, n0 + nb * 32, lane, ep_s[wave], (int)blockIdx.z);
     } else {
 #pragma unroll
         for (int nb = 0; nb < NB; ++nb)
diff --git a/canonicalvoting_amd/csrc/conv_rows_wp.hip b/canonicalvoting_amd/csrc/conv_rows_wp.hip
--- a/canonicalvoting_amd/csrc/conv_rows_wp.hip
+++ b/canonicalvoting_amd/csrc/conv_rows_wp.hip
@@ -219,7 +219,7 @@
     float (*ep)[EP_LD] = reinterpret_cast<float (*)[EP_LD]>(sm + wave * 32 * EP_LD * 4);
     if (a.wide) {
 #pragma unroll
-        for (int nb = 0; nb < NB; ++nb) epilogue_store_wide(a, acc[nb], rows_s + wave * 32, n0 + nb * 32, lane, ep);
+        for (int nb = 0; nb < NB; ++nb) epilogue_store_wide(a, acc[nb], rows_s + wave * 32, n0 + nb * 32, lane, ep, (int)blockIdx.z);
     } else {
 #pragma unroll
         for (int nb = 0; nb < NB; ++nb)
diff --git a/canonicalvoting_amd/csrc/net_exec.cpp b/canonicalvoting_amd/csrc/net_exec.cpp
--- a/canonicalvoting_amd/csrc/net_exec.cpp
+++ b/canonicalvoting_amd/csrc/net_exec.cpp
@@ -464,6 +464,7 @@
             d.perm_groups = o.perm_groups;
             d.perm_has_map = o.perm_groups > 1;
             if (plan_maps && d.perm_has_map && o.K == 27 && d.nbr) d.valid_words = d.nbr + out.rows * 27;
+            d.group_finish = plan_maps && o.perm_groups > 1;
         }
         int rc;
         if (nm) {
diff --git a/canonicalvoting_amd/csrc/sparse_conv.hip b/canonicalvoting_amd/csrc/sparse_conv.hip
--- a/canonicalvoting_amd/csrc/sparse_conv.hip
+++ b/canonicalvoting_amd/csrc/sparse_conv.hip
@@ -96,7 +96,7 @@
     }
     __syncthreads();
     float (*ep)[EP_LD] = reinterpret_cast<float (*)[EP_LD]>(w_s + wave * 32 * EP_LD * 4);
-    epilogue_store_wide(a, acc, rows_s + wave * 32, 0, lane, ep);
+    epilogue_store_wide(a, acc, rows_s + wave * 32, 0, lane, ep, (int)blockIdx.z);
 }
 
 template <class... MA>
@@ -220,11 +220,13 @@
 
 std::atomic<long long> g_opt_zskip{getenv("CV_ZSKIP") ? atoll(getenv("CV_ZSKIP")) : 1};
 std::atomic<long long> g_zskip_launches{0};
+std::atomic<long long> g_opt_group_finish{getenv("CV_GROUP_FINISH") ? atoll(getenv("CV_GROUP_FINISH")) : 0};
+std::atomic<long long> g_group_finish_launches{0};
 std::atomic<long long> g_opt_hd_mask{getenv("CV_HD") ? atoll(getenv("CV_HD")) : 4};
 std::atomic<long long> g_opt_hd_min_rows{getenv("CV_HD_MIN_ROWS") ? atoll(getenv("CV_HD_MIN_ROWS")) : 16384};
 std::atomic<long long> g_opt_hd_shape{getenv("CV_HD_SHAPE") ? atoll(getenv("CV_HD_SHAPE")) : 2};
 
-int launch_rows(ConvArgs a, const int NB, bool vec, hipStream_t st, ModelArgs* ma, int models) {
+int launch_rows(ConvArgs a, const int NB, bool vec, hipStream_t st, ModelArgs* ma, int models, bool group_finish) {
     dim3 grid((unsigned)((a.n_out + TM - 1) / TM), (unsigned)((a.cout + NB * 32 - 1) / (NB * 32)),
               (unsigned)a.splits);
     int per_wg = 0;
@@ -259,12 +261,34 @@
         const int hd_shape = (int)g_opt_hd_shape.load(std::memory_order_relaxed);
         const bool hd = NB <= 3 && ((hd_mask >> (NB - 1)) & 1) && a.n_out >= hd_min_rows;
         if (hd || !(a.splits > 1 && !a.perm_per_split && (long long)grid.x * grid.y <= CV_SPLIT_TICKETS)) a.tickets = nullptr;
-        if (hd) {
-            const int nw = hd_shape == 1 ? 4 : 8;
-            launch_conv_hd(a, NB, hd_shape, ma, dim3((unsigned)((a.n_out + nw * 32 - 1) / (nw * 32)), grid.y, grid.z), st);
-        } else {
-            launch_conv_hl(a, NB, ma, grid, st);
-        }
+        const int nw = hd_shape == 1 ? 4 : 8;
+        const auto launch = [&](const ConvArgs& x, unsigned gz) {
+            if (hd) launch_conv_hd(x, NB, hd_shape, ma, dim3((unsigned)((a.n_out + nw * 32 - 1) / (nw * 32)), grid.y, gz), st);
+            else launch_conv_hl(x, NB, ma, dim3(grid.x, grid.y, gz), st);
+        };
+        if (group_finish && a.perm_per_split && a.splits >= 2 && a.splits <= 4 && a.wide && !a.tickets &&
+            a.n_out * (long long)a.cout < (1ll << 30)) {
+            const int nj = a.j_end - a.j_begin;
+            int fin = 0;
+            while (fin + 1 < a.splits && (long long)nj * (fin + 1) / a.splits <= nj / 2) ++fin;
+            for (int k = 0; k < 4; ++k) {
+                a.gmask[k] = k < a.splits ? ~0u : 0u;
+                if (a.gvalid && k < a.splits) {
+                    const int jb = a.K * k / a.splits, je = a.K * (k + 1) / a.splits;
+                    a.gmask[k] = (unsigned)(((1ull << je) - 1) & ~((1ull << jb) - 1));
+                }
+            }
+            ConvArgs b = a;
+            a.group_hole = fin + 1;
+            b.group_fixed = fin + 1;
+            launch(a, (unsigned)a.splits - 1);
+            CV_LAUNCH_CHECK();
+            launch(b, 1u);
+            CV_LAUNCH_CHECK();
+            g_group_finish_launches.fetch_add(1, std::memory_order_relaxed);
+            return CV_OK;
+        }
+        launch(a, grid.z);
     } else if (vec && a.wp6 && per_wg <= WP_NPRE) {
         launch_conv_rows_wp(a, NB, a.pieces, false, grid, st);
     } else if (vec && a.wp6 && per_wg <= WP_NPRE_BIG) {
@@ -322,13 +346,14 @@
 static std::atomic<long long>* option_named(const char* name) {
     return !strcmp(name, "hd_mask") ? &g_opt_hd_mask : !strcmp(name, "hd_min_rows") ? &g_opt_hd_min_rows :
            !strcmp(name, "hd_shape") ? &g_opt_hd_shape : !strcmp(name, "zskip") ? &g_opt_zskip :
-           !strcmp(name, "zskip_launches") ? &g_zskip_launches : nullptr;
+           !strcmp(name, "zskip_launches") ? &g_zskip_launches : !strcmp(name, "group_finish") ? &g_opt_group_finish :
+           !strcmp(name, "group_finish_launches") ? &g_group_finish_launches : nullptr;
 }
 
 int cv_sp_set_option(const char* name, long long value, long long* previous) {
     CV_REQUIRE(name, CV_EINVAL, "null option name");
     std::atomic<long long>* o = option_named(name);
-    CV_REQUIRE(o, CV_EINVAL, "unknown option '%s' (hd_mask, hd_min_rows, hd_shape, zskip, zskip_launches)", name);
+    CV_REQUIRE(o, CV_EINVAL, "unknown option '%s' (hd_mask, hd_min_rows, hd_shape, zskip, zskip_launches, group_finish, group_finish_launches)", name);
     const long long before = o->exchange(value, std::memory_order_relaxed);
     if (previous) *previous = before;
     return CV_OK;
@@ -511,5 +536,6 @@
             a.partial = static_cast<float*>(d->ws);
         }
     }
-    return launch_rows(a, nb_for(d->cout), vec, st, pma, models);
-}
+    const bool group_finish = d->group_finish && d->perm_groups > 1 && g_opt_group_finish.load(std::memory_order_relaxed);
+    return launch_rows(a, nb_for(d->cout), vec, st, pma, models, group_finish);
+}
diff --git a/canonicalvoting_amd/csrc/sparse_conv_common.h b/canonicalvoting_amd/csrc/sparse_conv_common.h
--- a/canonicalvoting_amd/csrc/sparse_conv_common.h
+++ b/canonicalvoting_amd/csrc/sparse_conv_common.h
@@ -49,7 +49,17 @@
     int* tickets;
     const float* acc_scale_dev;
     const int* gvalid;
+    int group_hole;
+    int group_fixed;
+    unsigned gmask[4];
 };
+
+template <bool FIN>
+__device__ __forceinline__ int group_of(const ConvArgs& a) {
+    if constexpr (FIN) return a.group_fixed - 1;
+    const int z = (int)blockIdx.z;
+    return a.group_hole && z >= a.group_hole - 1 ? z + 1 : z;
+}
 
 struct ModelArgs {
     const cv_net_model_params* params;
@@ -153,6 +163,13 @@
     return make_float4(t[0], t[1], t[2], t[3]);
 }
 
+__device__ __forceinline__ float4 partial_load4_at(const float* base, unsigned long long uniform, unsigned offset) {
+    typedef const __attribute__((address_space(1))) unsigned char* gbytes;
+    typedef const __attribute__((address_space(1))) f32x4v* gvec;
+    const f32x4v t = __builtin_nontemporal_load((gvec)((gbytes)base + uniform + offset));
+    return make_float4(t[0], t[1], t[2], t[3]);
+}
+
 __device__ __forceinline__ void epilogue_apply1(const ConvArgs& a, long long row, int col, float v, float sc, float sh) {
     if (a.acc_in) v += a.acc_in[row * a.acc_ld + col];
     v = v * sc + sh;
@@ -209,7 +226,7 @@
 
 constexpr int EP_LD = 36;
 __device__ __forceinline__ __attribute__((used)) void epilogue_store_wide(const ConvArgs& a, const f32x16& acc, const int* rows, int colbase,
-                                                    int lane, float (*T)[EP_LD]) {
+                                                    int lane, float (*T)[EP_LD], int group) {
     const int h = lane >> 5, c = lane & 31;
 #pragma unroll
     for (int r = 0; r < 16; ++r) T[(r & 3) + 8 * (r >> 2) + 4 * h][c] = acc[r];
@@ -225,13 +242,71 @@
             if (row < 0) continue;
             float4 v = *reinterpret_cast<const float4*>(&T[rl][(lane & 7) * 4]);
             if (a.splits > 1) {
-                float* pp = a.partial + ((long long)blockIdx.z * a.n_out + row) * a.cout + col;
+                float* pp = a.partial + ((long long)group * a.n_out + row) * a.cout + col;
                 if (a.tickets) partial_store4_wt(pp, v);
                 else partial_store4(pp, v);
                 continue;
             }
             epilogue_apply4(a, row, col, v);
         }
+    }
+    __builtin_amdgcn_wave_barrier();
+}
+
+template <int BATCH = 4>
+__device__ __forceinline__ void epilogue_finish_wide(const ConvArgs& a, const f32x16& acc, const int* rows, int colbase,
+                                                     int lane, float (*T)[EP_LD], int group) {
+    const int h = lane >> 5, c = lane & 31;
+#pragma unroll
+    for (int r = 0; r < 16; ++r) T[(r & 3) + 8 * (r >> 2) + 4 * h][c] = acc[r];
+    __builtin_amdgcn_fence(__ATOMIC_RELEASE, "wavefront");
+    __builtin_amdgcn_wave_barrier();
+    __builtin_amdgcn_fence(__ATOMIC_ACQUIRE, "wavefront");
+    const int col = colbase + (lane & 7) * 4;
+    if (col < a.cout) {
+#pragma unroll
+      for (int it0 = 0; it0 < 4; it0 += BATCH) {
+        int row[BATCH];
+        unsigned w[BATCH], off[BATCH];
+#pragma unroll
+        for (int it = 0; it < BATCH; ++it) {
+            row[it] = rows[(lane >> 3) + 8 * (it0 + it)];
+            w[it] = row[it] < 0 ? 0u : a.gvalid ? (unsigned)a.gvalid[row[it]] : ~0u;
+            off[it] = ((unsigned)row[it] * (unsigned)a.cout + (unsigned)col) * 4u;
+        }
+        const auto mask_of = [&](int k) { return k == 0 ? a.gmask[0] : k == 1 ? a.gmask[1] : k == 2 ? a.gmask[2] : a.gmask[3]; };
+        const unsigned long long plane = (unsigned long long)a.n_out * (unsigned long long)a.cout * 4ull;
+        const unsigned m_own = mask_of(group);
+        float4 pv[BATCH][3];
+#pragma unroll
+        for (int it = 0; it < BATCH; ++it)
+#pragma unroll
+            for (int j = 0; j < 3; ++j) {
+                const int k = j + (j >= group ? 1 : 0);
+                pv[it][j] = make_float4(0.f, 0.f, 0.f, 0.f);
+                if (w[it] & mask_of(k))
+                    pv[it][j] = partial_load4_at(a.partial, k * plane, off[it]);
+            }
+#pragma unroll
+        for (int it = 0; it < BATCH; ++it) {
+            if (row[it] < 0) continue;
+            float4 own = *reinterpret_cast<const float4*>(&T[(lane >> 3) + 8 * (it0 + it)][(lane & 7) * 4]);
+            if (!(w[it] & m_own)) own = make_float4(0.f, 0.f, 0.f, 0.f);
+            const float4 t[4] = {group == 0 ? own : pv[it][0],
+                                 group == 1 ? own : group > 1 ? pv[it][1] : pv[it][0],
+                                 group == 2 ? own : group > 2 ? pv[it][2] : pv[it][1],
+                                 group == 3 ? own : pv[it][2]};
+            float4 sq[4];
+#pragma unroll
+            for (int k = 0; k < 4; ++k) {
+                sq[k] = make_float4(0.f, 0.f, 0.f, 0.f);
+                sq[k].x += t[k].x; sq[k].y += t[k].y; sq[k].z += t[k].z; sq[k].w += t[k].w;
+            }
+            const float4 x = make_float4(sq[0].x + sq[1].x + sq[2].x + sq[3].x, sq[0].y + sq[1].y + sq[2].y + sq[3].y,
+                                         sq[0].z + sq[1].z + sq[2].z + sq[3].z, sq[0].w + sq[1].w + sq[2].w + sq[3].w);
+            epilogue_apply4(a, row[it], col, x);
+        }
+      }
     }
     __builtin_amdgcn_wave_barrier();
 }
diff --git a/canonicalvoting_amd/me/__init__.py b/canonicalvoting_amd/me/__init__.py
--- a/canonicalvoting_amd/me/__init__.py
+++ b/canonicalvoting_amd/me/__init__.py
@@ -379,7 +379,7 @@
 def conv_forward(x_feats, weight, nbr, n_out, scale=None, shift=None, residual=None, relu=False,
                  out=None, flavour=0, row_perm=None, j_begin=0, j_end=0, acc_in=None, perm_groups=0,
                  cache_weights=True, pieces=None, in_hl=False, out_hl=False, res_hl=False, stem_mfma=False,
-                 split_tickets=None, weight_t=False, acc_scale_dev=None, step=None):
+                 split_tickets=None, weight_t=False, acc_scale_dev=None, step=None, group_finish=False):
     if pieces is None:
         pieces = 1 if COMPUTE_DTYPE == "bf16" else 3
     L = _lib.lib()
@@ -437,6 +437,8 @@
         d.split_tickets = split_tickets.data_ptr()
     if acc_scale_dev is not None:
         d.acc_scale_dev = acc_scale_dev.data_ptr()
+    if group_finish:
+        d.group_finish = 1
     with _on(dev):
         _lib.check(L.cv_sp_conv_f32(ctypes.byref(d), _stream(dev)), "cv_sp_conv_f32")
     return out
diff --git a/include/cv_hip.h b/include/cv_hip.h
--- a/include/cv_hip.h
+++ b/include/cv_hip.h
@@ -279,6 +279,7 @@
     int32_t* split_tickets;
     const float* acc_scale_dev;
     const int32_t* valid_words;
+    int group_finish;
 } cv_conv_desc;
 #define CV_SPLIT_TICKETS 4096
 
```
